# Nextomics/NextPolish2

Measured on AMD Instinct MI355X. Metric: polished reference Mbp/s (whole node) at 30x HiFi + k21/k31; FASTA identical to oracle, higher is better.
Workload: dtype u8

## Files before the change

### nextpolish2_amd/csrc/np2_batch.cpp

```cpp
#include "../../include/np2.h"
#include "np2_ctx.hpp"

#include <atomic>
#include <climits>
#include <cstring>
#include <condition_variable>
#include <mutex>
#include <thread>
#include <pthread.h>

#include <linux/futex.h>
#include <sys/syscall.h>
#include <unistd.h>

using namespace np2;

namespace {

struct Job {
    np2_contig *contig = nullptr;
    const np2_opts_t *opts = nullptr;
    uint8_t **out_bases = nullptr;
    uint32_t **out_pos = nullptr;
    uint64_t *out_len = nullptr;
    uint32_t *out_span = nullptr;
    int *rc = nullptr;
};

}

struct np2_batch {
    np2_ctx *parent = nullptr;
    int device = 0;
    hipStream_t stream = nullptr;
    std::vector<np2_ctx *> slots;
    std::vector<Recorder> recs;
    std::vector<std::thread> workers;
    std::string err;

    std::mutex mu;
    std::condition_variable cv_start, cv_done;
    uint64_t job_gen = 0;
    std::vector<Job> jobs;
    int n_running = 0;
    bool quit = false;

    std::mutex sync_mu;
    int n_active = 0, n_waiting = 0;
    std::atomic<uint32_t> flush_gen{0};
    std::atomic<bool> failed{false};
    std::string fail_msg;

    uint32_t *done_host = nullptr, *done_dev = nullptr;
    uint32_t done_seq = 0;
    std::atomic<uint32_t> issued_seq{0};
    std::atomic<uint32_t> done_pub{0};
    std::atomic<bool> spinner{false};
    double t_issued_last = 0;
    uint32_t wait_logged_seq = 0;

    bool time_diff = false;
    std::vector<std::pair<hipEvent_t, hipEvent_t>> diff_events;
    size_t diff_used = 0;
    float last_diff_ms = 0;
    int last_diff_launches = 0;
    uint64_t stat_launches = 0, stat_cmds = 0, stat_flushes = 0;
    double t_last_end = 0, ms_host = 0, ms_issue = 0, ms_wait = 0;
    std::vector<double> flush_log;
    double call_ms = 0, tail_ms = 0;
};

namespace {

inline void wait_generation(std::atomic<uint32_t> &gen, uint32_t seen) {
    static const double spin_us = getenv("NP2_BATCH_SPIN_US") ? atof(getenv("NP2_BATCH_SPIN_US")) : (wait_naps() ? 0.0 : 5.0);
    const double t_end = now_ms() + spin_us * 1e-3;
    for (;;) {
        for (int i = 0; i < 64; ++i) {
            if (gen.load(std::memory_order_acquire) != seen) return;
            __builtin_ia32_pause();
        }
        if (now_ms() >= t_end) break;
    }
    while (gen.load(std::memory_order_acquire) == seen)
        (void)syscall(SYS_futex, reinterpret_cast<uint32_t *>(&gen), FUTEX_WAIT_PRIVATE, seen, nullptr, nullptr, 0);
}
inline void publish_generation(std::atomic<uint32_t> &gen, uint32_t next) {
    gen.store(next, std::memory_order_release);
    (void)syscall(SYS_futex, reinterpret_cast<uint32_t *>(&gen), FUTEX_WAKE_PRIVATE, INT_MAX, nullptr, nullptr, 0);
}

__device__ __forceinline__ void k_flush_done(const uint32_t np2_bid, const uint32_t np2_nb, uint32_t *__restrict__ word, uint32_t seq) {
    if (threadIdx.x == 0) {
        __threadfence_system();
        __hip_atomic_store(word, seq, __ATOMIC_RELEASE, __HIP_MEMORY_SCOPE_SYSTEM);
    }
}

void flush(np2_batch *b) {
    const int n = (int)b->recs.size();
    const double t_begin = now_ms();
    double t_issued = t_begin;
    std::vector<size_t> idx(n, 0);
    hipStream_t s = b->stream;
    Recorder *saved = tl_recorder();
    tl_recorder() = nullptr;
    try {
        for (;;) {
            bool any = false;
            for (int i = 0; i < n; ++i) {
                auto &q = b->recs[i].q;
                while (idx[i] < q.size() && !q[idx[i]].kd) {
                    q[idx[i]].fn(s);
                    ++idx[i];
                    ++b->stat_cmds;
                }
                any |= idx[i] < q.size();
            }
            if (!any) break;
            const KernelDesc *best = nullptr;
            int best_n = 0, best_defer = 0;
            static constexpr size_t LOOKAHEAD = 8;
            for (int i = 0; i < n; ++i) {
                auto &q = b->recs[i].q;
                if (idx[i] >= q.size()) continue;
                const KernelDesc *kd = q[idx[i]].kd;
                bool seen = false;
                for (int j = 0; j < i && !seen; ++j)
                    seen = idx[j] < b->recs[j].q.size() && b->recs[j].q[idx[j]].kd == kd;
                if (seen) continue;
                int c = 0, defer = 0;
                for (int j = 0; j < n; ++j) {
                    auto &qj = b->recs[j].q;
                    if (idx[j] >= qj.size()) continue;
                    if (qj[idx[j]].kd == kd) {
                        ++c;
                        continue;
                    }
                    for (size_t k = idx[j] + 1; k < qj.size() && k <= idx[j] + LOOKAHEAD; ++k)
                        if (qj[k].kd == kd) {
                            ++defer;
                            break;
                        }
                }
                if (!best || defer < best_defer || (defer == best_defer && c > best_n)) best = kd, best_n = c, best_defer = defer;
            }
            uint32_t grids[MAXB];
            const void *args[MAXB];
            int m = 0;
            const bool timed = b->time_diff && strcmp(best->name, "k_diff_reads") == 0;
            auto issue = [&]() {
                if (!m) return;
                if (timed) {
                    if (b->diff_used == b->diff_events.size()) {
                        hipEvent_t e0 = nullptr, e1 = nullptr;
                        HIPCHK(hipEventCreate(&e0));
                        HIPCHK(hipEventCreate(&e1));
                        b->diff_events.push_back({e0, e1});
                    }
                    HIPCHK(hipEventRecord(b->diff_events[b->diff_used].first, s));
                }
                best->launch(s, m, grids, args);
                if (timed) {
                    HIPCHK(hipEventRecord(b->diff_events[b->diff_used].second, s));
                    ++b->diff_used;
                }
                ++b->stat_launches;
                m = 0;
            };
            for (int i = 0; i < n; ++i) {
                auto &r = b->recs[i];
                if (idx[i] >= r.q.size() || r.q[idx[i]].kd != best) continue;
                grids[m] = r.q[idx[i]].grid;
                args[m] = r.arena.data() + r.q[idx[i]].arg_off;
                ++m;
                ++idx[i];
                ++b->stat_cmds;
                if (m == best->max_batch) issue();
            }
            issue();
        }
        HIPCHK(hipGetLastError());
        const uint32_t seq = ++b->done_seq;
        NP2_LAUNCH(k_flush_done, 1, 64, s, b->done_dev, seq);
        t_issued = now_ms();
        b->issued_seq.store(seq, std::memory_order_release);
    } catch (const std::exception &ex) {
        b->fail_msg = ex.what();
        b->failed.store(true);
        (void)hipStreamSynchronize(s);
        for (np2_ctx *cx : b->slots) cx->lb_dirty = true, cx->h2d_inflight = false;
    }
    tl_recorder() = saved;
    for (auto &r : b->recs) r.clear();
    ++b->stat_flushes;
    b->ms_host += t_begin - b->t_last_end;
    b->ms_issue += t_issued - t_begin;
    b->flush_log.push_back(t_begin - b->t_last_end);
    b->flush_log.push_back(t_issued - t_begin);
    b->flush_log.push_back(0.0);
    b->t_last_end = t_issued;
    b->t_issued_last = t_issued;
}

void wait_done(np2_batch *b, uint32_t seq) {
    for (;;) {
        const uint32_t pub = b->done_pub.load(std::memory_order_acquire);
        if ((int32_t)(pub - seq) >= 0 || b->failed.load()) break;
        bool expected = false;
        if (b->spinner.compare_exchange_strong(expected, true)) {
            uint64_t spins = 0;
            uint32_t cur;
            HostWait hw;
            while ((int32_t)((cur = __atomic_load_n(b->done_host, __ATOMIC_ACQUIRE)) - seq) < 0) {
                if (b->failed.load()) break;
                if ((++spins & (wait_naps() ? 0xFFu : 0xFFFFu)) == 0) {
                    hipError_t e = hipStreamQuery(b->stream);
                    if (e != hipSuccess && e != hipErrorNotReady) {
                        b->fail_msg = std::string("device error during a batch flush: ") + hipGetErrorString(e);
                        b->failed.store(true);
                        break;
                    }
                    if (e == hipSuccess && (int32_t)(__atomic_load_n(b->done_host, __ATOMIC_ACQUIRE) - seq) < 0) {
                        b->fail_msg = "batch flush completed without posting";
                        b->failed.store(true);
                        break;
                    }
                }
                hw.pause();
            }
            b->spinner.store(false);
            publish_generation(b->done_pub, b->failed.load() ? pub + 1 : cur);
            if (b->failed.load()) return;
            continue;
        }
        wait_generation(b->done_pub, pub);
    }
    if (b->failed.load()) return;
    std::lock_guard<std::mutex> l(b->sync_mu);
    if (b->wait_logged_seq != seq && b->issued_seq.load() == seq && !b->flush_log.empty()) {
        const double t = now_ms();
        b->wait_logged_seq = seq;
        b->ms_wait += t - b->t_issued_last;
        b->flush_log.back() = t - b->t_issued_last;
        b->t_last_end = t;
    }
}

void group_sync(Recorder *r, bool need_done) {
    np2_batch *b = (np2_batch *)r->group;
    uint32_t my_gen;
    bool flushed = false;
    {
        std::lock_guard<std::mutex> l(b->sync_mu);
        my_gen = b->flush_gen.load(std::memory_order_relaxed);
        if (++b->n_waiting == b->n_active) {
            flush(b);
            b->n_waiting = 0;
            publish_generation(b->flush_gen, my_gen + 1);
            flushed = true;
        }
    }
    if (!flushed) wait_generation(b->flush_gen, my_gen);
    if (need_done && !b->failed.load()) wait_done(b, b->issued_seq.load(std::memory_order_acquire));
    if (b->failed.load()) throw Np2Error(NP2_E_DEVICE, "batch flush failed: " + b->fail_msg);
}

void leave_wave(np2_batch *b, Recorder *r) {
    std::lock_guard<std::mutex> l(b->sync_mu);
    if (!r->q.empty()) {
        np2_ctx *cx = b->slots[r->slot];
        cx->lb_dirty = true;
        cx->h2d_inflight = false;
    }
    r->clear();
    --b->n_active;
    if (b->n_active > 0 && b->n_waiting == b->n_active) {
        const uint32_t g = b->flush_gen.load(std::memory_order_relaxed);
        flush(b);
        b->n_waiting = 0;
        publish_generation(b->flush_gen, g + 1);
    }
}

void worker_main(np2_batch *b, int slot) {
    (void)hipSetDevice(b->device);
    (void)pthread_setname_np(pthread_self(), "np2-slot");
    uint64_t seen = 0;
    for (;;) {
        Job job;
        {
            std::unique_lock<std::mutex> l(b->mu);
            b->cv_start.wait(l, [&] { return b->quit || b->job_gen != seen; });
            if (b->quit) return;
            seen = b->job_gen;
            job = b->jobs[slot];
        }
        if (!job.contig) continue;
        Recorder *r = &b->recs[slot];
        tl_recorder() = r;
        int rc = np2_polish_resident(b->slots[slot], job.contig, job.opts, job.out_bases, job.out_pos, job.out_len);
        tl_recorder() = nullptr;
        for (auto &g : r->graveyard)
            dev_release_idle(g.first, (g.second >> 63) ? 0 : g.second, (g.second >> 63) ? (g.second & ~(1ull << 63)) : 0);
        r->graveyard.clear();
        leave_wave(b, r);
        if (rc == NP2_OK && job.out_span) (void)np2_last_span(b->slots[slot], &job.out_span[0], &job.out_span[1]);
        *job.rc = rc;
        {
            std::lock_guard<std::mutex> l(b->mu);
            if (--b->n_running == 0) b->cv_done.notify_all();
        }
    }
}

auto batch_sink(np2_batch *b) {
    return [b](int, const std::string &msg) { b->err = msg; };
}

}

extern "C" {

int np2_batch_create(np2_batch_t **out, np2_ctx_t *parent, int n_slots) {
    if (!out || !parent || n_slots < 1 || n_slots > 256) return NP2_E_ARG;
    *out = nullptr;
    return abi_guard([&] {
        std::unique_ptr<np2_batch, void (*)(np2_batch_t *)> b(new np2_batch(), np2_batch_destroy);
        b->parent = parent;
        b->device = parent->device;
        HIPCHK(hipSetDevice(b->device));
        HIPCHK(hipStreamCreateWithFlags(&b->stream, hipStreamNonBlocking));
        HIPCHK(hipHostMalloc((void **)&b->done_host, 256 * (size_t)(n_slots + 1), hipHostMallocMapped | hipHostMallocCoherent));
        memset(b->done_host, 0, 256 * (size_t)(n_slots + 1));
        HIPCHK(hipHostGetDevicePointer((void **)&b->done_dev, b->done_host, 0));
        b->recs.resize(n_slots);
        b->jobs.resize(n_slots);
        for (int i = 0; i < n_slots; ++i) {
            np2_ctx *cx = ctx_create_slot(parent, b->stream, b->done_host + 64 * (size_t)(i + 1), b->done_dev + 64 * (size_t)(i + 1));
            b->slots.push_back(cx);
            b->recs[i].group = b.get();
            b->recs[i].slot = i;
            b->recs[i].sync_fn = &group_sync;
        }
        for (int i = 0; i < n_slots; ++i) b->workers.emplace_back(worker_main, b.get(), i);
        *out = b.release();
        return NP2_OK;
    }, [parent](int, const std::string &msg) { parent->err = msg; });
}

void np2_batch_destroy(np2_batch_t *b) {
    if (!b) return;
    {
        std::lock_guard<std::mutex> l(b->mu);
        b->quit = true;
    }
    b->cv_start.notify_all();
    for (auto &t : b->workers) t.join();
    (void)hipSetDevice(b->device);
    if (b->stream) (void)hipStreamSynchronize(b->stream);
    {
        DevSyncScope idle;
        for (np2_ctx *cx : b->slots) np2_ctx_destroy(cx);
    }
    for (auto &e : b->diff_events) {
        (void)hipEventDestroy(e.first);
        (void)hipEventDestroy(e.second);
    }
    if (b->done_host) (void)hipHostFree(b->done_host);
    if (b->stream) (void)hipStreamDestroy(b->stream);
    delete b;
}

int np2_batch_set_priority(np2_batch_t *b, int high) {
    if (!b) return NP2_E_ARG;
    return abi_guard([&] {
        HIPCHK(hipSetDevice(b->device));
        int least = 0, greatest = 0;
        HIPCHK(hipDeviceGetStreamPriorityRange(&least, &greatest));
        HIPCHK(hipStreamSynchronize(b->stream));
        hipStream_t s = nullptr;
        HIPCHK(hipStreamCreateWithPriority(&s, hipStreamNonBlocking, high ? greatest : least));
        (void)hipStreamDestroy(b->stream);
        b->stream = s;
        for (np2_ctx *cx : b->slots) ctx_slot_set_stream(cx, s);
        return NP2_OK;
    }, batch_sink(b));
}

int np2_batch_slots(np2_batch_t *b) { return b ? (int)b->slots.size() : 0; }
np2_ctx_t *np2_batch_slot_ctx(np2_batch_t *b, int slot) {
    return (b && slot >= 0 && slot < (int)b->slots.size()) ? b->slots[slot] : nullptr;
}
const char *np2_batch_last_error(np2_batch_t *b) { return b ? b->err.c_str() : "null batch"; }
int np2_batch_set_sink(np2_batch_t *b, int slot, void *device_ptr, uint64_t cap) {
    if (!b || slot < 0 || slot >= (int)b->slots.size()) return NP2_E_ARG;
    b->slots[slot]->sink_dst = (uint8_t *)device_ptr;
    b->slots[slot]->sink_cap = device_ptr ? cap : 0;
    return NP2_OK;
}

int np2_batch_polish(np2_batch_t *b, np2_contig_t *const *contigs, int n, const np2_opts_t *opts, uint8_t **out_bases,
                     uint32_t **out_pos, uint64_t *out_len, uint32_t *out_span, int *rcs) {
    if (!b || !contigs || n < 0 || !opts || !out_len || !rcs) return NP2_E_ARG;
    return abi_guard([&] {
        const int S = (int)b->slots.size();
        int worst = NP2_OK;
        b->diff_used = 0;
        b->flush_log.clear();
        b->t_last_end = now_ms();
        const double t_call0 = b->t_last_end;
        for (int w0 = 0; w0 < n; w0 += S) {
            const int m = std::min(S, n - w0);
            {
                std::lock_guard<std::mutex> l(b->mu);
                for (int i = 0; i < S; ++i) {
                    Job j;
                    if (i < m) {
                        j.contig = contigs[w0 + i];
                        j.opts = opts;
                        j.out_bases = out_bases ? &out_bases[w0 + i] : nullptr;
                        j.out_pos = out_pos ? &out_pos[w0 + i] : nullptr;
                        j.out_len = &out_len[w0 + i];
                        j.out_span = out_span ? &out_span[2 * (w0 + i)] : nullptr;
                        j.rc = &rcs[w0 + i];
                    }
                    b->jobs[i] = j;
                }
                b->n_running = m;
                {
                    std::lock_guard<std::mutex> l2(b->sync_mu);
                    b->n_active = m;
                    b->n_waiting = 0;
                    b->failed.store(false);
                }
                ++b->job_gen;
            }
            b->cv_start.notify_all();
            {
                std::unique_lock<std::mutex> l(b->mu);
                b->cv_done.wait(l, [&] { return b->n_running == 0; });
            }
            for (int i = 0; i < m; ++i)
                if (rcs[w0 + i] != NP2_OK) {
                    worst = rcs[w0 + i];
                    b->err = std::string("contig ") + std::to_string(w0 + i) + ": " + np2_last_error(b->slots[i]);
                }
        }
        b->call_ms = now_ms() - t_call0;
        b->tail_ms = now_ms() - b->t_last_end;
        if (b->time_diff) {
            b->last_diff_ms = 0;
            b->last_diff_launches = (int)b->diff_used;
            for (size_t i = 0; i < b->diff_used; ++i) {
                float ms = 0;
                (void)hipEventSynchronize(b->diff_events[i].second);
                (void)hipEventElapsedTime(&ms, b->diff_events[i].first, b->diff_events[i].second);
                b->last_diff_ms += ms;
            }
        }
        return worst;
    }, batch_sink(b));
}

void np2_batch_set_timing(np2_batch_t *b, int enable) {
    if (b) b->time_diff = enable != 0;
}
int np2_batch_last_diff_ms(np2_batch_t *b, float *ms, int *launches) {
    if (!b || !ms || !launches) return NP2_E_ARG;
    *ms = b->last_diff_ms;
    *launches = b->last_diff_launches;
    return NP2_OK;
}
int np2_batch_last_call_ms(np2_batch_t *b, double *total_ms, double *tail_ms) {
    if (!b || !total_ms || !tail_ms) return NP2_E_ARG;
    *total_ms = b->call_ms;
    *tail_ms = b->tail_ms;
    return NP2_OK;
}
int np2_batch_flush_log(np2_batch_t *b, const double **log) {
    if (!b || !log) return 0;
    *log = b->flush_log.data();
    return (int)(b->flush_log.size() / 3);
}
int np2_batch_stats(np2_batch_t *b, uint64_t *launches, uint64_t *commands, uint64_t *flushes) {
    if (!b || !launches || !commands || !flushes) return NP2_E_ARG;
    *launches = b->stat_launches;
    *commands = b->stat_cmds;
    *flushes = b->stat_flushes;
    return NP2_OK;
}
}
```

### nextpolish2_amd/csrc/np2_cand.hip

```cpp
#include "np2_common.hpp"
#include "np2_kernels.hpp"
#include "np2_blockscan.hpp"
#include "np2_lookback.hpp"

namespace np2 {

template <int MODE>
__device__ __forceinline__ void k_scan_small(const uint32_t np2_bid, const uint32_t np2_nb, const uint32_t *__restrict__ in, uint32_t *__restrict__ out,
                                                     uint32_t n_host, const uint32_t *__restrict__ n_dev,
                                                     uint32_t *__restrict__ total_out, bool write_end) {
    __shared__ uint32_t sh[16];
    const uint32_t n = n_dev ? min(*n_dev, n_host) : n_host;
    uint32_t total;
    if (MODE == 2) {
        total = block_scan_array<OpMinI32>(
            n, sh, [&](uint32_t i) { return in[i]; },
            [&](uint32_t i, uint32_t pre, uint32_t v) { out[i] = OpMinI32::apply(pre, v); });
    } else {
        total = block_scan_array<OpAdd>(
            n, sh, [&](uint32_t i) { return in[i]; },
            [&](uint32_t i, uint32_t pre, uint32_t v) { out[i] = MODE == 0 ? pre : pre + v; });
    }
    if (threadIdx.x == 0) {
        if (MODE == 0 && write_end) out[n] = total;
// ... 103 lines not shown
    if (n > c) n -= c, col = 8, m = (uint32_t)(m64 >> 32);
    c = (uint32_t)__builtin_popcount(m & 0xFFFFu);
    if (n > c) n -= c, col += 4, m >>= 16;
    c = (uint32_t)__builtin_popcount(m & 0xFFu);
    if (n > c) n -= c, col += 2, m >>= 8;
    c = (uint32_t)__builtin_popcount(m & 0xFu);
    if (n > c) col += 1;
    return col;
}

__device__ uint32_t cand_measure(const CandCtx &cx, uint32_t r, const np2_read_t &rd, uint64_t ck_off, uint32_t start,
                                 uint32_t end, uint32_t &col_start) {
    uint32_t col_ck, t_ck;
    cand_anchor(cx, r, rd, ck_off, start, col_ck, t_ck);
    col_start = col_ck;
    if (end < t_ck) return 0;
    const uint32_t want_s = (start > t_ck ? start - t_ck : 0u) + 1;
    const uint32_t want_e = end + 1 - t_ck + 1;
    const uint8_t *base = cx.nib + rd.nib_off;
    const uint32_t n_cols = rd.n_cols;
    uint32_t seen = 0, len = 0;
    bool started = false;
    uint4 win = make_uint4(0, 0, 0, 0);
    uint32_t win_blk = 0xFFFFFFFFu;
    const uint64_t N1 = 0x1111111111111111ULL;
    for (uint32_t wi = col_ck >> 4;; ++wi) {
        const uint32_t c0 = wi << 4;
        if (c0 >= n_cols) break;
        if ((wi >> 1) != win_blk) {
            win_blk = wi >> 1;
            win = *reinterpret_cast<const uint4 *>(base + ((size_t)win_blk << 4));
        }
        const uint32_t r0 = (wi & 1) ? win.z : win.x, r1 = (wi & 1) ? win.w : win.y;
        const uint64_t w = (uint64_t)(((r0 & 0x0F0F0F0Fu) << 4) | ((r0 >> 4) & 0x0F0F0F0Fu)) |
                           ((uint64_t)(((r1 & 0x0F0F0F0Fu) << 4) | ((r1 >> 4) & 0x0F0F0F0Fu)) << 32);
        uint64_t valid = N1;
        if (c0 < col_ck) valid &= ~((1ULL << (4 * (col_ck - c0))) - 1ULL);
        if (n_cols - c0 < 16) valid &= (1ULL << (4 * (n_cols - c0))) - 1ULL;
        uint64_t nonins = (~(w >> 3)) & valid;
        if (c0 == 0) nonins |= valid & 1ULL;
        const uint64_t x = (w & 0x7777777777777777ULL) ^ 0x4444444444444444ULL;
        const uint64_t nongap = (x | (x >> 1) | (x >> 2)) & valid;
        const uint32_t cn = (uint32_t)__builtin_popcountll(nonins);
        uint32_t lo = 0, hi = 16;
        bool done = false;
        if (!started && seen + cn >= want_s) {
            lo = nth_col16(nonins, want_s - seen);
            col_start = c0 + lo;
            started = true;
        }
        if (seen + cn >= want_e) {
            hi = nth_col16(nonins, want_e - seen);
            done = true;
        }
        if (started) {
            uint64_t m = nongap;
            if (lo) m &= ~((1ULL << (4 * lo)) - 1ULL);
            if (hi < 16) m &= (1ULL << (4 * hi)) - 1ULL;
            len += (uint32_t)__builtin_popcountll(m);
        }
        seen += cn;
        if (done) break;
    }
    return started ? len : 0u;
}

struct NibReader {
    const uint8_t *base;
    uint64_t w;
    uint32_t wbase;
    __device__ __forceinline__ uint8_t get(uint32_t c) {
        const uint32_t b = c & ~15u;
        if (b != wbase) {
            const uint2 v = *reinterpret_cast<const uint2 *>(base + (b >> 1));
            const uint32_t x = ((v.x & 0x0F0F0F0Fu) << 4) | ((v.x >> 4) & 0x0F0F0F0Fu);
            const uint32_t y = ((v.y & 0x0F0F0F0Fu) << 4) | ((v.y >> 4) & 0x0F0F0F0Fu);
            w = (uint64_t)x | ((uint64_t)y << 32);
            wbase = b;
        }
        return (uint8_t)((w >> (4 * (c & 15))) & 15);
    }
};

__device__ void cand_write(const CandCtx &cx, uint32_t r, const np2_read_t &rd, uint32_t pj, uint32_t g, uint32_t col, uint32_t t,
                           uint32_t len, uint8_t *__restrict__ seq_out, uint64_t *kmer_out) {
    const uint8_t *base = cx.nib + rd.nib_off;
    const uint32_t limit = cx.lq_end[pj] + cx.ksize;
    bool have_kmer = false;
    if (col + cx.ksize <= rd.n_cols) {
        const uint32_t k = cx.ksize, W0 = col >> 4, sh = (col & 15) * 4;
        auto ld = [&](uint32_t W) -> uint64_t {
            const uint2 v = *reinterpret_cast<const uint2 *>(base + ((size_t)W << 3));
            const uint32_t x = ((v.x & 0x0F0F0F0Fu) << 4) | ((v.x >> 4) & 0x0F0F0F0Fu);
            const uint32_t y = ((v.y & 0x0F0F0F0Fu) << 4) | ((v.y >> 4) & 0x0F0F0F0Fu);
            return (uint64_t)x | ((uint64_t)y << 32);
        };
        const uint64_t x0 = ld(W0), x1 = ld(W0 + 1), x2 = ld(W0 + 2);
        uint64_t lo = sh ? (x0 >> sh) | (x1 << (64 - sh)) : x0, hi = sh ? (x1 >> sh) | (x2 << (64 - sh)) : x1;
        auto nmask = [](uint32_t n) -> uint64_t { return n >= 16 ? ~0ULL : ((1ULL << (4 * n)) - 1ULL); };
        const uint64_t N1 = 0x1111111111111111ULL;
        const uint32_t avail = min(32u, rd.n_cols - col);
        const uint64_t a_lo = nmask(avail), a_hi = avail > 16 ? nmask(avail - 16) : 0ULL;
        const uint64_t ng_lo = ~(lo >> 2) & N1 & a_lo, ng_hi = ~(hi >> 2) & N1 & a_hi;
        const uint32_t c_lo = (uint32_t)__builtin_popcountll(ng_lo);
        if (c_lo + (uint32_t)__builtin_popcountll(ng_hi) >= k) {
            uint32_t kk = k, C = 0;
            uint64_t m = ng_lo;
            if (kk > c_lo) kk -= c_lo, C = 16, m = ng_hi;
            uint32_t c = (uint32_t)__builtin_popcount((uint32_t)m);
            if (kk > c) kk -= c, C += 8, m >>= 32;
            uint32_t m32 = (uint32_t)m;
            c = (uint32_t)__builtin_popcount(m32 & 0xFFFFu);
            if (kk > c) kk -= c, C += 4, m32 >>= 16;
            c = (uint32_t)__builtin_popcount(m32 & 0xFFu);
            if (kk > c) kk -= c, C += 2, m32 >>= 8;
            c = (uint32_t)__builtin_popcount(m32 & 0xFu);
            if (kk > c) C += 1;
            const uint64_t u_lo = nmask(C + 1), u_hi = C + 1 > 16 ? nmask(C + 1 - 16) : 0ULL;
            const uint64_t hi4_lo = (lo >> 2) & N1 & u_lo, hi4_hi = (hi >> 2) & N1 & u_hi;
            const bool plain = (((lo | (lo >> 1)) & hi4_lo) | ((hi | (hi >> 1)) & hi4_hi)) == 0;
            const uint64_t r_lo = nmask(C) & ~0xFULL, r_hi = C > 16 ? nmask(C - 16) : 0ULL;
            const uint32_t ins = (uint32_t)__builtin_popcountll(lo & r_lo & 0x8888888888888888ULL) +
                                 (uint32_t)__builtin_popcountll(hi & r_hi & 0x8888888888888888ULL);
            const uint32_t steps = C ? C - 1 : 0u;
            if (plain && t + (steps - ins) <= limit) {
                lo &= u_lo, hi &= u_hi;
                uint64_t g_lo = hi4_lo, g_hi = hi4_hi;
                while (g_lo | g_hi) {
                    if (g_lo) {
                        const uint64_t below = (g_lo & (0 - g_lo)) - 1;
                        lo = (lo & below) | (((lo >> 4) | (hi << 60)) & ~below);
                        g_lo = ((g_lo >> 4) | (g_hi << 60)) & ~below;
                        hi >>= 4;
                        g_hi >>= 4;
                    } else {
                        const uint64_t below = (g_hi & (0 - g_hi)) - 1;
                        hi = (hi & below) | ((hi >> 4) & ~below);
                        g_hi = (g_hi >> 4) & ~below;
                    }
                }
                auto squeeze = [](uint64_t x) -> uint64_t {
                    uint64_t y = x & 0x3333333333333333ULL;
                    y = (y | (y >> 2)) & 0x0F0F0F0F0F0F0F0FULL;
                    y = (y | (y >> 4)) & 0x00FF00FF00FF00FFULL;
                    y = (y | (y >> 8)) & 0x0000FFFF0000FFFFULL;
                    return (y | (y >> 16)) & 0xFFFFFFFFULL;
                };
                const uint64_t mask = (1ULL << (2 * (uint64_t)k)) - 1;
                const uint64_t codes = (squeeze(lo) | (squeeze(hi) << 32)) & mask;
                uint64_t rb = __builtin_bitreverse64(codes);
                rb = ((rb >> 1) & 0x5555555555555555ULL) | ((rb & 0x5555555555555555ULL) << 1);
                const uint64_t fw = rb >> (64 - 2 * k), rv = ~codes & mask;
                *kmer_out = yak_hash64(fw < rv ? fw : rv, mask);
                have_kmer = true;
            }
        }
    }
    if (!have_kmer) {
        NibReader nr{base, 0, 0xFFFFFFFFu};
        const uint64_t ksize = cx.ksize, shift = 2 * (ksize - 1), mask = (1ULL << (2 * ksize)) - 1;
        uint64_t fw = 0, rv = 0, l = 0;
        for (uint32_t c = col; c < rd.n_cols && l < ksize; ++c) {
            const uint8_t nb = nr.get(c);
            if (c != col && !(nb & 8)) ++t;
            const uint8_t q = nb & 7;
            if (q != 4) {
                fw = ((fw << 2) | (uint64_t)q) & mask;
// ... 301 lines not shown
        n_blk, sh, [&](uint32_t i) { return blk_sum[2 * n_blk + i]; }, [&](uint32_t, uint32_t, uint32_t) {});
    if (threadIdx.x == 0) {
        cand_off[n_reg] = ta;
        reg_soff[n_reg] = tb;
        *n_cand = ta;
        *n_bytes = tb;
        *grow = tc;
    }
}

__device__ __forceinline__ void k_cand_offsets_lb(const uint32_t np2_bid, const uint32_t np2_nb, Lookback lb, uint32_t n_blocks, const uint32_t *__restrict__ blk_sum,
                                                         uint32_t n_blk, uint32_t n_reg, uint32_t *__restrict__ blk_coff,
                                                         uint32_t *__restrict__ blk_soff, uint32_t *__restrict__ cand_off,
                                                         uint32_t *__restrict__ reg_soff, uint32_t *__restrict__ n_cand,
                                                         uint32_t *__restrict__ n_bytes, uint32_t *__restrict__ grow,
                                                         uint32_t *__restrict__ err) {
    __shared__ uint32_t sh[8];
    const uint32_t bid = lb_block_id(lb, sh);
    const uint32_t i0 = (bid * 256 + threadIdx.x) * 4;
    uint32_t a[4], b[4], sa = 0, sb = 0;
#pragma unroll
    for (uint32_t k = 0; k < 4; ++k) {
        a[k] = i0 + k < n_blk ? blk_sum[i0 + k] : 0u;
        b[k] = i0 + k < n_blk ? blk_sum[n_blk + i0 + k] : 0u;
        sa += a[k];
        sb += b[k];
    }
    uint32_t ta, tb, pa, pb;
    uint32_t ra = block_excl_scan<OpAdd, 4>(sa, sh, ta);
    uint32_t rb = block_excl_scan<OpAdd, 4>(sb, sh, tb);
    lb_exclusive2(lb, bid, ta, tb, sh, err, pa, pb);
    ra += pa, rb += pb;
#pragma unroll
    for (uint32_t k = 0; k < 4; ++k)
        if (i0 + k < n_blk) {
            blk_coff[i0 + k] = ra;
            blk_soff[i0 + k] = rb;
            ra += a[k];
            rb += b[k];
        }
    if (bid == n_blocks - 1 && threadIdx.x == 255) {
        cand_off[n_reg] = ra;
        reg_soff[n_reg] = rb;
        *n_cand = ra;
        *n_bytes = rb;
    }
    if (bid == 0) {
        uint32_t c = 0, tc;
        for (uint32_t i = threadIdx.x; i < n_blk; i += 256) c += blk_sum[2 * n_blk + i];
        (void)block_excl_scan<OpAdd, 4>(c, sh, tc);
        if (threadIdx.x == 0) *grow = tc;
    }
}

static constexpr uint32_t MERGE_LB_BLOCKS = 32;
__device__ __forceinline__ void k_lq_merge_scan_lb(const uint32_t np2_bid, const uint32_t np2_nb, Lookback lb, const uint32_t *__restrict__ raw_start,
                                                   const uint32_t *__restrict__ raw_end, const uint32_t *__restrict__ n_raw, uint32_t n_host,
                                                   uint32_t *__restrict__ headflag, uint32_t *__restrict__ hidx, uint32_t *__restrict__ err) {
    __shared__ uint32_t sh[16];
    const uint32_t bid = lb_block_id(lb, sh);
    const uint32_t n = min(*n_raw, n_host);
    const uint32_t seg = ((n + MERGE_LB_BLOCKS - 1) / MERGE_LB_BLOCKS + 1023u) & ~1023u;
    const uint32_t lo = min(bid * seg, n), hi = min(lo + seg, n);
    auto flag = [&](uint32_t j) { return (j >= 1 && raw_end[j] >= raw_start[j - 1]) ? 0u : 1u; };
    uint32_t cnt = 0;
    for (uint32_t j = lo + threadIdx.x; j < hi; j += 1024) cnt += flag(j);
    uint32_t total, pre, dummy;
    (void)block_excl_scan<OpAdd, 16>(cnt, sh, total);
    lb_exclusive2(lb, bid, total, 0u, sh, err, pre, dummy);
    uint32_t carry = pre;
    for (uint32_t j0 = lo; j0 < hi; j0 += 1024) {
        const uint32_t j = j0 + threadIdx.x;
        const uint32_t v = j < hi ? flag(j) : 0u;
        uint32_t tot;
        const uint32_t ex = block_excl_scan<OpAdd, 16>(v, sh, tot);
        if (j < hi) {
            hidx[j] = carry + ex;
            headflag[j] = v;
        }
        carry += tot;
    }
}

__device__ __forceinline__ void k_region_write(const uint32_t np2_bid0, const uint32_t np2_nb, CandCtx cx, uint32_t n_reg, const uint32_t *__restrict__ kept_read,
                                                      const uint32_t *__restrict__ kept_len,
                                                      const uint32_t *__restrict__ kept_col,
                                                      const uint32_t *__restrict__ reg_ncand,
                                                      const uint32_t *__restrict__ reg_bytes,
                                                      const uint32_t *__restrict__ blk_coff,
                                                      const uint32_t *__restrict__ blk_soff,
                                                      uint32_t *__restrict__ cand_off, uint32_t *__restrict__ reg_soff,
                                                      uint32_t cand_cap,
                                                      uint32_t seq_cap, uint32_t *__restrict__ cand_order,
                                                      uint64_t *__restrict__ cand_kmer, uint32_t *__restrict__ cand_seq_off,
                                                      uint8_t *__restrict__ cand_seq) {
    const uint32_t np2_bid = xcd_order(np2_bid0, np2_nb);
    __shared__ __attribute__((aligned(4))) uint8_t s_str[RM_REG][CLEAN_MAX_LEN];
    __shared__ uint64_t s_km[RM_REG];
    __shared__ uint32_t s_so[RM_REG][64];
    __shared__ uint32_t s_oc[RM_REG];
    __shared__ uint32_t s_q[4][RM_RPW * 64];
    const uint32_t lane = threadIdx.x & 63, wv = (uint32_t)__builtin_amdgcn_readfirstlane((int)(threadIdx.x >> 6));
    const uint32_t g0 = (np2_bid * 4 + wv) * RM_RPW, mb0 = g0 / 4;
    uint32_t nq = 0;
    uint32_t oc = 0, ob = 0;
    if (g0 < n_reg) oc = blk_coff[mb0], ob = blk_soff[mb0];
    uint32_t clean_h = 0;
    uint32_t my_len[RM_RPW], my_so[RM_RPW], my_ci[RM_RPW];
    bool my_clean[RM_RPW];
    uint32_t n[RM_RPW], rb[RM_RPW], st[RM_RPW], ln0[RM_RPW];
#pragma unroll
    for (uint32_t h = 0; h < RM_RPW; ++h) {
        const uint32_t g = g0 + h;
        n[h] = 0, rb[h] = 0, st[h] = 0, ln0[h] = 0;
        if (g < n_reg) n[h] = reg_ncand[g], rb[h] = reg_bytes[g], st[h] = cx.lq_start[g], ln0[h] = cx.lq_end[g] - st[h] + 1;
    }
    uint32_t len[RM_RPW], col[RM_RPW], rd_[RM_RPW], refc[RM_RPW];
#pragma unroll
    for (uint32_t h = 0; h < RM_RPW; ++h) {
        const size_t ks = (size_t)(g0 + h) * LQSEQ_MAX_CAN_COUNT + lane;
        const bool act = lane < n[h];
        len[h] = act ? kept_len[ks] : 0u;
        col[h] = act ? kept_col[ks] : 0u;
        rd_[h] = act ? kept_read[ks] : 0u;
        const uint32_t p = st[h] + lane;
        refc[h] = (n[h] && lane < ln0[h] && ln0[h] <= CLEAN_MAX_LEN) ? cx.refnib[p >> 3] >> (4 * (p & 7)) : 0u;
    }
#pragma unroll
    for (uint32_t h = 0; h < RM_RPW; ++h) {
        const uint32_t g = g0 + h, slot = wv * RM_RPW + h;
        my_len[h] = 0, my_so[h] = 0, my_ci[h] = 0, my_clean[h] = false;
        if (g >= n_reg) continue;
        if (g == n_reg - 1 && lane == 0 && cand_off[n_reg] < cand_cap) cand_seq_off[cand_off[n_reg]] = reg_soff[n_reg];
        if (lane == 0) {
            cand_off[g] = oc;
            reg_soff[g] = ob;
            s_oc[slot] = oc;
        }
        const bool act = lane < n[h];
        const uint32_t so = ob + wave_excl(len[h]);
        const uint32_t ci = oc + lane;
        const bool ok = act && ci < cand_cap && (uint64_t)so + len[h] <= seq_cap;
        if (ok) {
            cand_order[ci] = rd_[h];
            cand_seq_off[ci] = so;
        }
        const bool clean = ok && col[h] == CAND_CLEAN;
        const uint64_t cm = __ballot(clean);
        const bool queued = ok && (!clean || (lane == 0 && rd_[h] == 0));
        my_len[h] = len[h], my_so[h] = so, my_ci[h] = ci, my_clean[h] = clean && !queued;
        s_so[slot][lane] = so;
        if (cm) {
            clean_h |= 1u << h;
            if (lane < ln0[h]) s_str[slot][lane] = (uint8_t)((0x54474341u >> (8 * (refc[h] & 3))) & 0xFFu);
        }
        const uint64_t dq = __ballot(queued);
        if (queued) s_q[wv][nq + lanes_below(dq)] = (slot << 6) | lane;
        nq += (uint32_t)__builtin_popcountll(dq);
        oc += n[h];
        ob += rb[h];
    }
    wave_lds_sync();
    for (uint32_t e = lane; e < nq; e += 64) {
        const uint32_t w = s_q[wv][e], slot = w >> 6, li = w & 63;
        const uint32_t g = (np2_bid * 4 + slot / RM_RPW) * RM_RPW + slot % RM_RPW;
        const size_t ks = (size_t)g * LQSEQ_MAX_CAN_COUNT + li;
        const uint32_t r = kept_read[ks], len = kept_len[ks];
        uint32_t col = kept_col[ks];
        const ReadInfo ri = cx.rinfo[r];
        const np2_read_t rd = rinfo_read(ri);
        const uint32_t t0 = max(cx.lq_start[g], rd.aln_t_s);
        if (col == CAND_CLEAN) col = t0;
        const uint32_t ci = s_oc[slot] + li;
        uint64_t km;
        cand_write(cx, r, rd, ri.pj, g, col, t0, len, cand_seq + s_so[slot][li], &km);
        cand_kmer[ci] = km;
        if (li == 0 && r == 0) s_km[slot] = km;
    }
    wave_lds_sync();
#pragma unroll
    for (uint32_t h = 0; h < RM_RPW; ++h) {
        if (!((clean_h >> h) & 1u)) continue;
        const uint32_t slot = wv * RM_RPW + h;
        if (my_clean[h]) {
            cand_kmer[my_ci[h]] = s_km[slot];
            typedef uint32_t u32_any __attribute__((aligned(1)));
            uint8_t *dst = cand_seq + my_so[h];
            const uint32_t L4 = my_len[h] & ~3u;
            for (uint32_t j = 0; j < L4; j += 4) *reinterpret_cast<u32_any *>(dst + j) = *reinterpret_cast<const uint32_t *>(&s_str[slot][j]);
            for (uint32_t j = L4; j < my_len[h]; ++j) dst[j] = s_str[slot][j];
        }
    }
}

void launch_scan_small_excl(hipStream_t s, const uint32_t *in, uint32_t *out, uint32_t n, const uint32_t *n_dev,
                            uint32_t *total_out, bool write_end) {
    NP2_LAUNCH(k_scan_small<0>, dim3(1), 1024, s, in, out, n, n_dev, total_out, write_end);
}
void launch_scan_lb_excl(hipStream_t s, const Lookback &lb, const uint32_t *in, uint32_t *out, uint32_t n, bool write_end,
                          uint32_t *err) {
    const uint32_t nb = scan_lb_blocks(n);
    NP2_LAUNCH(k_scan_lb_excl, dim3(nb), SCAN_LB_THREADS, s, lb, nb, in, out, n, write_end, err);
}
void launch_scan_lb_popc(hipStream_t s, const Lookback &lb, const uint32_t *bits, uint32_t *out, uint32_t n_words, uint32_t *err) {
    const uint32_t nb = scan_lb_blocks((uint64_t)n_words + 1);
    NP2_LAUNCH(k_scan_lb_popc, dim3(nb), SCAN_LB_THREADS, s, lb, nb, bits, out, n_words + 1, false, err);
}
uint32_t scan_lb_blocks(uint64_t n) { return (uint32_t)std::max<uint64_t>(1, (n + SCAN_LB_BLOCK - 1) / SCAN_LB_BLOCK); }
void launch_scan_small_incl(hipStream_t s, const int32_t *in, int32_t *out, uint32_t n, const uint32_t *n_dev) {
    NP2_LAUNCH(k_scan_small<1>, dim3(1), 1024, s, (const uint32_t *)in, (uint32_t *)out, n, n_dev, (uint32_t *)nullptr, false);
}
void launch_scan_small_min(hipStream_t s, const int32_t *in, int32_t *out, uint32_t n, const uint32_t *n_dev) {
    NP2_LAUNCH(k_scan_small<2>, dim3(1), 1024, s, (const uint32_t *)in, (uint32_t *)out, n, n_dev, (uint32_t *)nullptr, false);
}
static CandCtx mk_cand(const CandPtrs &c) {
    return CandCtx{c.reads, c.nib,    c.ck_off, c.ckpt,        c.lq_start, c.lq_end, c.pj,
                   c.pcount, c.alive, c.rinfo, c.tile_rd_off, c.tile_rd, c.n_tiles,  c.ksize,
                   c.rec_key, c.rec_read, c.tile_n, c.rec_pidx, c.bucket_cap, c.refnib, c.L};
}
void launch_region_measure(hipStream_t s, const CandPtrs &c, uint32_t n_reg, uint32_t *kept_read, uint32_t *kept_len,
                           uint32_t *kept_col, uint32_t *reg_ncand, uint32_t *reg_bytes, uint32_t *reg_maxlen,
                           uint32_t *blk_sum) {
    if (n_reg)
        NP2_LAUNCH_WAVES(k_region_measure, RM_WAVES, dim3((n_reg + RM_REG - 1) / RM_REG), 256, s,
                         mk_cand(c), n_reg, kept_read, kept_len, kept_col, reg_ncand, reg_bytes, reg_maxlen, blk_sum);
}
uint32_t cand_offsets_blocks(uint32_t n_reg) { return ((n_reg + 3) / 4 + 1023) / 1024; }
void launch_cand_offsets(hipStream_t s, const uint32_t *blk_sum, uint32_t n_reg, uint32_t *blk_coff, uint32_t *blk_soff,
                         uint32_t *cand_off, uint32_t *reg_soff, uint32_t *n_cand, uint32_t *n_bytes, uint32_t *grow,
                         const Lookback *lb, uint32_t *err) {
    if (lb)
        NP2_LAUNCH(k_cand_offsets_lb, dim3(cand_offsets_blocks(n_reg)), 256, s, *lb, cand_offsets_blocks(n_reg), blk_sum, (n_reg + 3) / 4, n_reg, blk_coff, blk_soff, cand_off, reg_soff, n_cand, n_bytes, grow, err);
    else
        NP2_LAUNCH(k_cand_offsets, dim3(1), 1024, s, blk_sum, (n_reg + 3) / 4, n_reg, blk_coff, blk_soff, cand_off, reg_soff, n_cand, n_bytes, grow);
}
void launch_lq_merge_scan_lb(hipStream_t s, const Lookback &lb, const uint32_t *raw_start, const uint32_t *raw_end, const uint32_t *n_raw,
                             uint32_t n_host, uint32_t *headflag, uint32_t *hidx, uint32_t *err) {
    NP2_LAUNCH(k_lq_merge_scan_lb, dim3(MERGE_LB_BLOCKS), 1024, s, lb, raw_start, raw_end, n_raw, n_host, headflag, hidx, err);
}
uint32_t lq_merge_lb_blocks() { return MERGE_LB_BLOCKS; }
void launch_region_write(hipStream_t s, const CandPtrs &c, uint32_t n_reg, const uint32_t *kept_read,
                         const uint32_t *kept_len, const uint32_t *kept_col, const uint32_t *reg_ncand,
                         const uint32_t *reg_bytes, const uint32_t *blk_coff, const uint32_t *blk_soff, uint32_t *cand_off,
                         uint32_t *reg_soff, uint32_t cand_cap, uint32_t seq_cap, uint32_t *cand_order, uint64_t *cand_kmer,
                         uint32_t *cand_seq_off, uint8_t *cand_seq) {
    if (n_reg)
        NP2_LAUNCH(k_region_write, dim3((n_reg + RM_REG - 1) / RM_REG), 256, s, mk_cand(c), n_reg, kept_read, kept_len, kept_col, reg_ncand, reg_bytes, blk_coff, blk_soff, cand_off, reg_soff, cand_cap, seq_cap, cand_order, cand_kmer, cand_seq_off, cand_seq);
}

}
```

### nextpolish2_amd/csrc/np2_host.cpp

```cpp
#include "../../include/np2.h"
#include "np2_common.hpp"
#include "np2_kernels.hpp"
#include "np2_ctx.hpp"
#include "np2_phase_host.hpp"

#include <algorithm>
#include <atomic>
#include <thread>
#include <chrono>
#include <cstdio>
#include <cstdlib>
#include <cstring>
#include <map>
#include <mutex>
#include <stdexcept>
#include <string>
#include <unordered_map>
#include <unordered_set>
#include <future>
#include <functional>
#include <vector>

using namespace np2;

// ... 130 lines not shown
            off_own.assign(off, off + R + 1);
            edges_own.assign(edges, edges + off[R]);
            off = off_own.data(), edges = edges_own.data();
        }
        if (!view_key) return;
        pair_key.assign(view_key, view_key + view_n);
        pair_cnt.assign(view_cnt, view_cnt + view_n);
        view_key = nullptr, view_cnt = nullptr, view_n = 0;
    }
    std::vector<uint32_t> first_key;
    std::vector<int32_t> ref_w;
    std::vector<uint8_t> ref_seen, bad;
    const uint8_t *d_bad = nullptr;
    bool key_added = false;
};

bool vote_rows_from_pairs(VoteData &vd, bool use_all) {
    const uint32_t R = vd.R;
    const uint64_t *k = vd.keys();
    const uint32_t *cn = vd.cnts();
    const uint64_t np = vd.n_pairs();
    std::vector<uint32_t> n_lo(R, 0), n_up(R, 0);
    uint32_t nokey = 0;
    auto listed = [&](uint64_t i, uint32_t &a, uint32_t &b) {
        a = (uint32_t)(k[i] >> 32), b = (uint32_t)k[i];
        if (a >= R || b >= R || vd.first_key[a] == 0xFFFFFFFFu || vd.first_key[b] == 0xFFFFFFFFu) return false;
        return use_all || !(vd.bad[a] | vd.bad[b]);
    };
    for (uint64_t i = 0; i < np; ++i) {
        uint32_t a = (uint32_t)(k[i] >> 32), b = (uint32_t)k[i];
        if (b <= a || b - a - 1 >= EDGE_BAND || (i && k[i - 1] >= k[i])) return false;
        if (a >= R || b >= R || vd.first_key[a] == 0xFFFFFFFFu || vd.first_key[b] == 0xFFFFFFFFu) ++nokey;
        if (listed(i, a, b)) ++n_lo[b], ++n_up[a];
    }
    vd.off_own.assign((size_t)R + 1, 0);
    std::vector<uint32_t> cur_lo(R), cur_up(R);
    for (uint32_t v = 0; v < R; ++v) {
        cur_lo[v] = vd.off_own[v], cur_up[v] = vd.off_own[v] + n_lo[v];
        vd.off_own[v + 1] = cur_up[v] + n_up[v];
    }
    vd.edges_own.resize(vd.off_own[R]);
    for (uint64_t i = 0; i < np; ++i) {
        uint32_t a, b;
        if (!listed(i, a, b)) continue;
        const int32_t same = (int32_t)(cn[i] & 0xFFFFu), neg = (int32_t)(cn[i] >> 16);
        const float w = (float)(neg >= 3 ? -neg : same - neg);
        vd.edges_own[cur_lo[b]++] = phase::Graph::Edge(a, w);
        vd.edges_own[cur_up[a]++] = phase::Graph::Edge(b, w);
    }
    vd.off = vd.off_own.data(), vd.edges = vd.edges_own.data(), vd.n_nokey = nokey;
    return true;
}

void vote_collect(np2_ctx *cx, np2_contig *c, PassCounts &pc, bool asref, bool use_all, int pass, uint32_t own_lo,
                  uint32_t own_hi, VoteData &vd, bool wide = false, uint64_t key_add = 0) {
    hipStream_t s = cx->stream;
    const uint32_t R = c->R, n_reg = pc.n_reg;
    RegionTables rt = region_tables(cx, n_reg);
    uint32_t NE = 0, NU = 0;
    vd = VoteData();
    vd.R = R;
    {
        EventTimer t(cx, "vote_phase");
        cx->reg_lable.ensure(n_reg + 2);
        cx->grp.ensure((size_t)pc.NC_cap + 2);
        cx->ecount.ensure(n_reg + 2);
        cx->eoff.ensure(std::max<size_t>(n_reg + 2, (size_t)c->L + 2));
        const size_t RP = ((size_t)R + 63) & ~(size_t)63;
        const size_t band_words = (size_t)R * EDGE_BAND;
        const size_t b_v = RP * 10, b_off = (((size_t)R + 2) * 4 + 15) & ~(size_t)15;
        uint8_t *vbuf;
        uint32_t *row_off;
        if (wide) {
            cx->votebuf.ensure(b_v);
            cx->band_off.ensure((size_t)R + 2);
            vbuf = cx->votebuf.p, row_off = cx->band_off.p;
        } else {
            cx->votepack.ensure(b_v + b_off + band_words * 2 * sizeof(phase::Graph::Edge) + 64);
            vbuf = cx->votepack.p, row_off = (uint32_t *)(cx->votepack.p + b_v);
        }
        uint32_t *v_first = (uint32_t *)vbuf;
        int32_t *v_refw = (int32_t *)(vbuf + RP * 4);
        uint8_t *v_seen = vbuf + RP * 8, *v_bad = vbuf + RP * 9;
        op_fill(cx, v_first, 0xFF, RP * 4);
        op_fill(cx, v_refw, 0, RP * 6);
        launch_vote_phase(s, rt, asref, use_all, cx->lq_start.p, own_lo, own_hi, cx->reg_lable.p, cx->grp.p, cx->ecount.p,
                          v_refw, v_seen, v_bad, v_first, cx->scal.p + S_ERR);
        exclusive_total_n(cx, cx->ecount.p, cx->eoff.p, n_reg);
        launch_vote_counts(s, v_first, v_bad, R, cx->scal.p + S_M1);
        cx->band.ensure(band_words + 4);
        cx->band_n.ensure((size_t)R + 2);
        op_fill(cx, cx->scal.p + S_M3, 0, 4);
        launch_edges_row(s, rt, cx->grp.p, cx->ecount.p, cx->pj.p, cx->pcount.p, cx->alive.p, R, cx->band.p, cx->band_n.p,
                         cx->scal.p + S_M3);
        if (wide) {
            exclusive_total_n(cx, cx->band_n.p, row_off, R);
            cx->ekey.ensure(band_words + 2);
            cx->eval.ensure(band_words + 2);
            launch_band_emit(s, cx->band.p, R, row_off, cx->ekey.p, cx->eval.p, cx->scal.p + S_NRAW, key_add);
        } else {
            cx->row_cnt.ensure((size_t)R + 2);
            launch_vote_rows_count(s, cx->band.p, cx->band_n.p, v_bad, use_all, R, cx->row_cnt.p, cx->scal.p + S_NOKEY);
            exclusive_total_n(cx, cx->row_cnt.p, row_off, R);
            launch_vote_rows_emit(s, cx->band.p, cx->band_n.p, v_bad, use_all, v_first, R, row_off, cx->votepack.p + b_v + b_off,
                                  cx->scal.p + S_NRAW, cx->scal.p + S_NOKEY);
        }
    }
    const size_t RP = ((size_t)R + 63) & ~(size_t)63;
    const size_t b_v = RP * 10, b_off = (((size_t)R + 2) * 4 + 15) & ~(size_t)15;
    auto per_read = [&](const uint8_t *vb) {
        vd.first_key.assign((const uint32_t *)vb, (const uint32_t *)vb + R);
        vd.ref_w.assign((const int32_t *)(vb + RP * 4), (const int32_t *)(vb + RP * 4) + R);
        vd.ref_seen.assign(vb + RP * 8, vb + RP * 8 + R);
        vd.bad.assign(vb + RP * 9, vb + RP * 9 + R);
    };
    bool far = false, have_per_read = false;
    {
        std::vector<uint32_t> sc;
        uint8_t *pin = nullptr;
        const size_t EB = sizeof(phase::Graph::Edge);
        static_assert(sizeof(phase::Graph::Edge) == 8 && alignof(phase::Graph::Edge) <= 8, "an edge is {u32 neighbour, f32 weight}");
        const uint32_t likely = (uint32_t)std::min<size_t>((size_t)R * EDGE_BAND * 2, std::max<size_t>((size_t)R * 128, 1u << 15));
        if (wide) {
            sc = fetch_scal(cx, cx->scal.p + S_M0, cx->eoff.p + n_reg);
        } else {
            pin = (uint8_t *)cx->pin_d2h.ensure(b_v + b_off + (size_t)likely * EB + 64);
            const uint32_t seq = ++cx->mbox_seq;
            launch_post(cx->stream, cx->scal.p, S_COUNT, cx->mbox_dev, seq, cx->scal.p + S_M0, cx->eoff.p + n_reg, nullptr, nullptr,
                        nullptr, nullptr, nullptr, nullptr, nullptr, nullptr);
            op_d2h(cx, pin, cx->votepack.p, b_v + b_off);
            launch_copy_counted(cx->stream, (uint32_t *)(pin + b_v + b_off), (const uint32_t *)(cx->votepack.p + b_v + b_off),
                                (const uint32_t *)(cx->votepack.p + b_v) + R, likely * (uint32_t)(EB / 4), (uint32_t)(EB / 4));
            op_sync(cx);
            if (__atomic_load_n(&cx->mbox_host[0], __ATOMIC_ACQUIRE) != seq)
                throw Np2Error(NP2_E_DEVICE, "mailbox not posted after a synchronisation");
            sc.assign(cx->mbox_host + 1, cx->mbox_host + 1 + S_COUNT);
        }
        check_region_err(cx, sc[S_ERR]);
        pc.resolve(sc);
        NE = sc[S_M0];
        if (!cx->trace && sc[S_M1] == 0 && sc[S_M2] == 0) {
            if (NE) throw Np2Error(NP2_E_DEVICE, "internal: pair edges without voting reads");
            return;
        }
        NU = sc[S_NRAW];
        far = sc[S_M3] != 0 || cx->hooks.edge_sort;
        if (!wide) cx->timing.host.push_back({far ? "vote_sort" : "vote_rows", 1.0f});
        if (!wide) {
            per_read(pin);
            have_per_read = true;
            vd.d_bad = cx->votepack.p + RP * 9;
            if (!far) {
                if (NU > likely) {
                    pin = (uint8_t *)cx->pin_d2h.ensure(b_v + b_off + (size_t)NU * EB + 64);
                    op_d2h(cx, pin, cx->votepack.p, b_v + b_off + (size_t)NU * EB);
                    op_sync(cx);
                }
                vd.off = (const uint32_t *)(pin + b_v), vd.edges = (const phase::Graph::Edge *)(pin + b_v + b_off);
                vd.n_nokey = sc[S_NOKEY];
                if (vd.off[R] != NU) throw Np2Error(NP2_E_DEVICE, "internal: vote rows and edge count disagree");
            }
        }
    }
    vd.any = true;
    if (NE && far) {
        {
            EventTimer t(cx, "vote_phase");
            cx->ekey.ensure(NE + 2);
            cx->ekey_s.ensure(NE + 2);
            cx->eval.ensure(NE + 2);
            cx->eval_s.ensure(NE + 2);
            cx->eflag.ensure(NE + 2);
            cx->eidx.ensure(NE + 2);
            cx->ew.ensure(NE + 2);
            cx->tmp.ensure(prim_temp_bytes((size_t)NE + 2));
            launch_edges_write(s, rt, cx->reg_lable.p, cx->grp.p, cx->ecount.p, cx->eoff.p, cx->ekey.p, cx->eval.p);
            unsigned rbits = 1;
            while ((1ull << rbits) < (uint64_t)R + 1) ++rbits;
            prim_op(cx, [=](hipStream_t st) {
                if (prim_sort_pairs_u64_u32(st, cx->tmp.p, cx->tmp.cap, cx->ekey.p, cx->ekey_s.p, cx->eval.p, cx->eval_s.p, NE,
                                            32 + rbits))
                    throw Np2Error(NP2_E_DEVICE, "rocprim edge sort failed");
            });
            launch_edge_reduce(s, cx->ekey_s.p, cx->eval_s.p, NE, cx->eflag.p, (uint32_t *)cx->ew.p);
            exclusive_total(cx, cx->eflag.p, cx->eidx.p, NE);
            launch_edge_compact(s, cx->ekey_s.p, cx->eflag.p, cx->eidx.p, (const uint32_t *)cx->ew.p, NE, cx->ekey.p,
                                cx->eval.p, cx->scal.p + S_NRAW);
            NU = fetch_scal(cx)[S_NRAW];
        }
    } else if (!NE) {
        NU = 0;
    }
    if (wide || far) {
        const size_t b_key = ((size_t)NU * 8 + 15) & ~(size_t)15, b_w = ((size_t)NU * 4 + 15) & ~(size_t)15;
        const size_t b_pr = have_per_read ? 0 : b_v;
        uint8_t *pin = (uint8_t *)cx->pin_d2h.ensure(b_key + b_w + b_pr + 64);
        if (tl_recorder()) {
            cx->votepack2.ensure(b_key + b_w + b_pr + 64);
            op_copy_d2d(cx, cx->votepack2.p, cx->ekey.p, (size_t)NU * 8);
            op_copy_d2d(cx, cx->votepack2.p + b_key, cx->eval.p, (size_t)NU * 4);
            if (b_pr) op_copy_d2d(cx, cx->votepack2.p + b_key + b_w, cx->votebuf.p, b_pr);
            op_d2h(cx, pin, cx->votepack2.p, b_key + b_w + b_pr);
        } else {
            op_d2h(cx, pin, cx->ekey.p, (size_t)NU * 8);
            op_d2h(cx, pin + b_key, cx->eval.p, (size_t)NU * 4);
            if (b_pr) op_d2h(cx, pin + b_key + b_w, cx->votebuf.p, b_pr);
        }
        op_sync(cx);
        vd.view_key = (const uint64_t *)pin, vd.view_cnt = (const uint32_t *)(pin + b_key), vd.view_n = NU;
        vd.key_added = wide && !far;
        if (b_pr) {
            per_read(pin + b_key + b_w);
            if (wide) vd.d_bad = cx->votebuf.p + RP * 9;
        }
    }
// ... 554 lines not shown
            fprintf(stderr, "\n");
        }
        const bool wide = n_tiles >= 2048;
        Lookback lb{};
        if (wide) lb = next_lookback(cx, tile_scan_blocks(n_tiles));
        launch_tile_offsets(s, cx->tile_nn.p, cx->tile_nr.p, n_tiles, cx->tile_noff.p, cx->tile_roff.p, M_p, n_lq,
                            cx->scal.p + S_BEST, S_NLQ + 1 - S_BEST, wide ? &lb : nullptr, cx->scal.p + S_ERR,
                            (const long long *)cx->tile_gain.p, (unsigned long long *)(cx->scal.p + S_PFGAIN0));
        launch_pf_compact(s, n_tiles, cx->pf_slots.p, cx->tile_scan.p, cx->tile_nn.p, cx->tile_noff.p, cx->tile_roff.p,
                          cx->cns_pos.p, cx->cns_base.p, cx->cns_cls.p, cx->lq_nothead.p, cx->lq_list.p, cb.lq_cap,
                          cx->scal.p + S_ERR, cx->scal.p + S_PF, cx->scal.p + S_PFOUT, cx->scal.p + S_NBAD, cx->scal.p + S_NBAD2);
    }
    lq_regions_issue(cx, cb, M_p, n_lq);
}

void pass_front_issue(np2_ctx *cx, np2_contig *c, uint32_t T, int pass, bool force_unfused = false) {
    cx->front_fused = !force_unfused && front_can_fuse(cx);
    if (!cx->front_fused || cx->trace) {
        uint32_t n_nodes = 0, n_runs = 0;
        {
            WallTimer w(cx, "wall_graph");
            build_graph(cx, c, T, n_nodes, n_runs);
        }
        trace_graph(cx, c, pass, n_nodes);
        if (!cx->front_fused) {
            consensus_and_regions_issue(cx, c, n_nodes, n_runs, T);
            return;
        }
    }
    pass_front_fused_issue(cx, c, T);
}
void consensus_and_regions_finish(np2_ctx *cx, np2_contig *c, uint32_t T, int pass, uint32_t &M, uint32_t &n_reg, bool whole_contig = true) {
    const uint32_t *M_p = cx->eoff.p + c->L;
    std::vector<uint32_t> sc = fetch_scal(cx, cx->scal.p + S_M0, M_p);
    if (cx->front_fused) {
        const int64_t total = (int64_t)(((uint64_t)sc[S_PFGAIN1] << 32) | sc[S_PFGAIN0]);
        const int64_t end_rel = (int64_t)(((uint64_t)sc[S_PFEND1] << 32) | sc[S_PFEND0]);
        const bool negative = end_rel <= SCORE_NEG / 2 || total + end_rel < 0;
        if (sc[S_PFOUT] & PF_NEED_BIG) cx->pf_big = true;
        if ((sc[S_PFOUT] & PF_REDO) || negative) {
            ++cx->front_redos;
            cx->timing.host.push_back({"front_redo", 1.0f});
            pass_front_issue(cx, c, T, pass, true);
            sc = fetch_scal(cx, cx->scal.p + S_M0, M_p);
        }
    }
    check_region_err(cx, sc[S_ERR]);
    if (!cx->front_fused && sc[S_BEST] == 0xFFFFFFFFu && !whole_contig)
        throw Np2Error(NP2_E_UNSUPPORTED,
                       "best path score is negative at the end of a shard (the reference's default node is chosen by the whole "
                       "contig's score): polish this contig unsharded");
    M = sc[S_M0];
    if (M == 0) throw Np2Error(NP2_E_REFPANIC, "reference would panic: empty consensus");
    n_reg = sc[S_NRAW] ? sc[S_NREG] : 0;
}

void extract_candidates(np2_ctx *cx, np2_contig *c, uint32_t n_reg, uint16_t min_kmer_count, int pass,
                        PassCounts &pc) {
    hipStream_t s = cx->stream;
    const uint32_t R = c->R;
    REFPANIC_IF(cx->yaks.empty(), "index out of bounds: opt.yak[0]");
    if ((uint64_t)n_reg * LQSEQ_MAX_CAN_COUNT >= 0xFFFFFFF0ull) throw Np2Error(NP2_E_NOMEM, "too many LQ regions");
    const uint32_t NC_cap = n_reg * LQSEQ_MAX_CAN_COUNT;
    static const uint64_t exact_from = getenv("NP2_CAND_EXACT_FROM") ? strtoull(getenv("NP2_CAND_EXACT_FROM"), nullptr, 10) : (1ull << 28);
    const bool exact_bytes = c->n_cols >= exact_from && !cx->trace;
    uint32_t SB_cap = (uint32_t)std::min<uint64_t>(c->n_cols + 64, 0xFFFFFFF0ull);
    cx->mval.ensure(R + 2);
    cx->smin.ensure(R + 2);
    cx->pj.ensure(R + 2);
    cx->pcount.ensure(R + 2);
    cx->rinfo.ensure(R + 2);
    cx->reg_ncand.ensure(n_reg + 2);
    cx->reg_bytes.ensure(n_reg + 2);
    cx->reg_soff.ensure(n_reg + 2);
    cx->reg_maxlen.ensure(n_reg + 2);
    cx->blk_sum.ensure(3 * ((size_t)n_reg / 4 + 2));
    cx->blk_coff.ensure((size_t)n_reg / 4 + 2);
    cx->blk_soff.ensure((size_t)n_reg / 4 + 2);
    cx->cand_off.ensure(n_reg + 2);
    cx->kept_read.ensure((size_t)NC_cap + 2);
    cx->kept_len.ensure((size_t)NC_cap + 2);
    cx->kept_col.ensure((size_t)NC_cap + 2);
    cx->cand_order.ensure((size_t)NC_cap + 2);
    cx->cand_kmer.ensure((size_t)NC_cap + 2);
    cx->cand_seq_off.ensure((size_t)NC_cap + 2);
    if (!exact_bytes) cx->cand_seq.ensure((size_t)SB_cap + 64);
    cx->kscore.ensure((size_t)NC_cap + 2);
    cx->long_list.ensure((size_t)NC_cap + 2);
    CandPtrs cp{c->reads.p,   c->nib.p,   c->ck_off.p,      c->ckpt.p,    cx->lq_start.p, cx->lq_end.p, cx->pj.p,
                cx->pcount.p, cx->alive.p, cx->rinfo.p, c->tile_rd_off.p, c->tile_rd.p, c->n_tiles, cx->yaks[0].k,
                cx->keys_raw.p, cx->vals_raw.p, cx->tile_n.p,
                (cx->pidx_valid && cx->bucket_cap) ? cx->tile_pidx.p : nullptr, cx->bucket_cap,
                (const uint32_t *)c->refnib.p, c->L};
    {
        EventTimer t(cx, "candidates");
        launch_read_m(s, c->reads.p, R, cx->alive.p, cx->lq_start.p, n_reg, cx->mval.p);
        scan_incl_min(cx, cx->mval.p, cx->smin.p, R);
        launch_pair_count(s, c->reads.p, R, cx->alive.p, cx->lq_start.p, cx->lq_end.p, n_reg, cx->smin.p, cx->pj.p,
                          cx->pcount.p, c->ck_off.p, cx->rinfo.p);
        launch_region_measure(s, cp, n_reg, cx->kept_read.p, cx->kept_len.p, cx->kept_col.p, cx->reg_ncand.p,
                              cx->reg_bytes.p, cx->reg_maxlen.p, cx->blk_sum.p);
        {
            const bool wide = n_reg > 0;
            Lookback lb{};
            if (wide) lb = next_lookback(cx, cand_offsets_blocks(n_reg));
            launch_cand_offsets(s, cx->blk_sum.p, n_reg, cx->blk_coff.p, cx->blk_soff.p, cx->cand_off.p, cx->reg_soff.p,
                                cx->scal.p + S_NC, cx->scal.p + S_SB, cx->scal.p + S_GROW, wide ? &lb : nullptr,
                                cx->scal.p + S_ERR);
        }
        if (exact_bytes) {
            const std::vector<uint32_t> sc = fetch_scal(cx);
            check_region_err(cx, sc[S_ERR]);
            pc.resolve(sc);
            SB_cap = (uint32_t)std::min<uint64_t>((uint64_t)pc.SB + 64, SB_cap);
            cx->cand_seq.ensure((size_t)SB_cap + 64);
        }
        launch_region_write(s, cp, n_reg, cx->kept_read.p, cx->kept_len.p, cx->kept_col.p, cx->reg_ncand.p,
                            cx->reg_bytes.p, cx->blk_coff.p, cx->blk_soff.p, cx->cand_off.p, cx->reg_soff.p, NC_cap + 1,
                            SB_cap, cx->cand_order.p, cx->cand_kmer.p, cx->cand_seq_off.p, cx->cand_seq.p);
    }
    {
        EventTimer t(cx, "kmer_score");
        launch_cand_score(s, cx->yaks[0].dev(), cx->cand_seq_off.p, cx->cand_seq.p, cx->cand_kmer.p, cx->scal.p + S_NC,
                          NC_cap, min_kmer_count, cx->kscore.p, cx->long_list.p, cx->scal.p + S_NLONG);
    }
    pc.n_reg = n_reg;
    pc.NC_cap = NC_cap;
    pc.SB_cap = SB_cap;
    pc.known = exact_bytes;
    if (cx->trace) pc.resolve(fetch_scal(cx));
    trace_region_tables(cx, pass, "cand", pc, false);
}

Cns fetch_cns(np2_ctx *cx, uint32_t M) {
    Cns c;
    c.pos = d2h(cx, cx->cns_pos.p, M);
    c.base = d2h(cx, cx->cns_base.p, M);
    return c;
}

struct ResultOut {
    uint8_t *bases = nullptr;
    uint32_t *pos = nullptr;
    uint64_t len = 0;
    bool want_pos = true;
    bool want_bases = true;
    void release() {
        if (bases) pinned_pool().put(bases), bases = nullptr;
        if (pos) pinned_pool().put(pos), pos = nullptr;
    }
};
void fetch_result(np2_ctx *cx, const uint32_t *dpos, const uint8_t *dbase, const uint32_t *M_p, uint32_t M_cap, ResultOut &r,
                  uint32_t M_likely = 0xFFFFFFFFu) {
    const double t0 = now_ms();
    std::vector<uint32_t> sc;
    if (cx->sink_dst && cx->sink_cap) launch_copy_len(cx->stream, cx->sink_dst, dbase, M_p, 1, cx->sink_cap);
    if (r.want_bases || r.want_pos) {
        const uint32_t seq = ++cx->mbox_seq;
        launch_post(cx->stream, cx->scal.p, S_COUNT, cx->mbox_dev, seq, cx->scal.p + S_M0, M_p, nullptr, nullptr, nullptr, nullptr,
                    nullptr, nullptr, dpos, cx->scal.p + S_M1);
        if (r.want_bases) r.bases = (uint8_t *)pinned_pool().get((size_t)M_cap + 1);
        if (r.want_pos) r.pos = (uint32_t *)pinned_pool().get(((size_t)M_cap + 1) * 4);
        if ((r.want_bases && !r.bases) || (r.want_pos && !r.pos)) throw Np2Error(NP2_E_NOMEM, "pinned result allocation failed");
        uint32_t first = std::min(M_cap, M_likely);
        const bool exact_b = r.want_bases && op_d2h_len(cx, r.bases, dbase, M_p, 1, M_cap);
        const bool exact_p = r.want_pos && op_d2h_len(cx, r.pos, dpos, M_p, 4, (size_t)M_cap * 4);
        if (r.want_bases && !exact_b) op_d2h(cx, r.bases, dbase, first);
        if (r.want_pos && !exact_p) op_d2h(cx, r.pos, dpos, (size_t)first * 4);
        if ((exact_b || !r.want_bases) && (exact_p || !r.want_pos)) first = M_cap;
        op_sync(cx);
        if (__atomic_load_n(&cx->mbox_host[0], __ATOMIC_ACQUIRE) != seq)
            throw Np2Error(NP2_E_DEVICE, "mailbox not posted after a synchronisation");
        sc.assign(cx->mbox_host + 1, cx->mbox_host + 1 + S_COUNT);
        if (sc[S_M0] > first && sc[S_M0] <= M_cap) {
            const uint32_t rest = sc[S_M0] - first;
            if (r.want_bases) op_d2h(cx, r.bases + first, dbase + first, rest);
            if (r.want_pos) op_d2h(cx, r.pos + first, dpos + first, (size_t)rest * 4);
            op_sync(cx);
        }
    } else {
        sc = fetch_scal(cx, cx->scal.p + S_M0, M_p, nullptr, nullptr, nullptr, nullptr, nullptr, nullptr, dpos, cx->scal.p + S_M1);
    }
    check_region_err(cx, sc[S_ERR]);
    const uint32_t M = sc[S_M0];
    if (M == 0) throw Np2Error(NP2_E_REFPANIC, "reference would panic: empty consensus");
    if (M > M_cap) throw Np2Error(NP2_E_DEVICE, "internal: consensus longer than its bound");
    r.len = M;
    cx->last_first_pos = sc[S_M1];
    cx->last_last_pos = sc[S_M2];
    cx->last_dbase = dbase;
    cx->last_dpos = dpos;
    cx->last_len = M;
    if (cx->stage_timing) cx->timing.host.push_back({"wall_fetch_result", (float)(now_ms() - t0)});
}

struct PolishRun {
    np2_ctx *cx = nullptr;
    np2_contig *c = nullptr;
    np2_opts_t o{};
    uint32_t own_lo = 0, own_hi = 0xFFFFFFFFu;
    uint32_t T = 0, pass = 0, M = 0, n_reg = 0;
    bool reuse = false;
    bool front_issued = false;
    uint32_t grow_prev = 0xFFFFFFFFu;
    bool wide_votes = false;
    uint64_t key_add = 0;
    PassCounts pc;
    bool final_pass() const { return pass + 1 == o.iter_count; }
};

void run_begin(PolishRun &r) {
    np2_ctx *cx = r.cx;
    if (r.o.iter_count < 1) throw Np2Error(NP2_E_ARG, "iter_count must be >= 1");
    HIPCHK(hipSetDevice(cx->device));
    cx->trace_items.clear();
    cx->last_dbase = nullptr;
    cx->last_dpos = nullptr;
    cx->scal.ensure(SCAL_TOTAL);
    cx->alive.ensure(r.c->R + 2);
    {
        WallTimer w(cx, "wall_diff");
        run_diff(cx, r.c, r.T);
    }
    launch_init_alive(cx->stream, r.c->reads.p, r.c->R, cx->alive.p);
    r.pass = 0;
    r.reuse = false;
}

void run_pass_front(PolishRun &r) {
    np2_ctx *cx = r.cx;
    np2_contig *c = r.c;
    if (!r.reuse) {
        {
            WallTimer w(cx, "wall_cns_lq");
            if (!r.front_issued) pass_front_issue(cx, c, r.T, (int)r.pass);
            r.front_issued = false;
            consensus_and_regions_finish(cx, c, r.T, (int)r.pass, r.M, r.n_reg, !r.wide_votes);
        }
        if (cx->trace) {
            trace_cns(cx, (int)r.pass, "cns_raw", fetch_cns(cx, r.M));
            trace_put(cx, (int)r.pass, "lq.start", d2h(cx, cx->lq_start.p, r.n_reg));
            trace_put(cx, (int)r.pass, "lq.end", d2h(cx, cx->lq_end.p, r.n_reg));
        }
    }
    if (r.n_reg == 0) return;
    if (!r.reuse) {
        r.pc = PassCounts();
        r.pc.M = r.M;
        WallTimer w(cx, "wall_extract");
        extract_candidates(cx, c, r.n_reg, r.o.min_kmer_count, (int)r.pass, r.pc);
    } else if (r.pc.NC_cap) {
        op_copy_d2d(cx, cx->kscore.p, cx->kscore_saved.p, (size_t)(r.pc.known ? r.pc.NC : r.pc.NC_cap) * 2);
// ... 1192 lines not shown
```

### nextpolish2_amd/csrc/np2_kernels.hip

```cpp
#include "np2_common.hpp"
#include "np2_kernels.hpp"
#include "np2_blockscan.hpp"
#include "np2_nib128.hpp"
#include "../../include/np2.h"

namespace np2 {

__device__ __forceinline__ uint8_t ref_code(const uint8_t *__restrict__ refnib, uint32_t p) {
    return (refnib[p >> 1] >> (4 * (p & 1))) & 7;
}

__device__ __forceinline__ void k_encode_ref(const uint32_t np2_bid, const uint32_t np2_nb, const uint8_t *__restrict__ read0, uint32_t L, uint8_t *__restrict__ refnib,
                             uint32_t nbytes_total, uint32_t stride, uint32_t *__restrict__ err) {
    uint32_t i = np2_bid * blockDim.x + threadIdx.x;
    if (i >= nbytes_total) return;
    uint32_t c0 = 2 * i, c1 = 2 * i + 1;
    uint8_t b = c0 < L ? read0[i] : 0;
    uint8_t hi = c0 < L ? (b >> 4) : 0, lo = c1 < L ? (b & 15) : 0;
    if ((c0 < L && c0 != 0 && (hi & 8)) || (c1 < L && (lo & 8))) atomicOr(err, 1u);
    if (c0 < L && (hi & 7) == 7) atomicOr(err, 1u);
    if (c1 < L && (lo & 7) == 7) atomicOr(err, 1u);
    refnib[i] = (uint8_t)((hi & 7) | ((lo & 7) << 4));
    const uint8_t nx = c1 + 1 < L ? (uint8_t)((read0[i + 1] >> 4) & 7) : (uint8_t)0;
    refnib[stride + i] = (uint8_t)(((hi & 7) << 4) | (lo & 7));
    refnib[2 * (size_t)stride + i] = (uint8_t)(((lo & 7) << 4) | nx);
}

__device__ __forceinline__ void k_post(const uint32_t np2_bid, const uint32_t np2_nb, uint32_t *__restrict__ scal, uint32_t n_scal, uint32_t *__restrict__ mbox, uint32_t seq,
                       uint32_t *__restrict__ dst0, const uint32_t *__restrict__ src0, uint32_t *__restrict__ dst1,
                       const uint32_t *__restrict__ src1, uint32_t *__restrict__ dst2, const uint32_t *__restrict__ src2,
                       uint32_t *__restrict__ dst3, const uint32_t *__restrict__ src3,
                       const uint32_t *__restrict__ ends_of, uint32_t *__restrict__ ends_dst) {
    if (threadIdx.x == 0) {
        if (dst0) *dst0 = *src0;
        if (dst1) *dst1 = *src1;
        if (dst2) *dst2 = *src2;
        if (dst3) *dst3 = *src3;
        if (ends_of) {
            const uint32_t n = *dst0;
            ends_dst[0] = n ? ends_of[0] : 0u;
            ends_dst[1] = n ? ends_of[n - 1] : 0u;
        }
    }
    __threadfence();
    if (threadIdx.x < n_scal)
        mbox[1 + threadIdx.x] = __hip_atomic_load(&scal[threadIdx.x], __ATOMIC_RELAXED, __HIP_MEMORY_SCOPE_AGENT);
    __threadfence_system();
    if (threadIdx.x == 0) __hip_atomic_store(&mbox[0], seq, __ATOMIC_RELEASE, __HIP_MEMORY_SCOPE_SYSTEM);
}
__device__ __forceinline__ void k_fill(const uint32_t np2_bid, const uint32_t np2_nb, uint8_t *__restrict__ p, uint64_t n, uint32_t v4) {
    const uint64_t o = ((uint64_t)np2_bid * 256 + threadIdx.x) * 16;
    if (o >= n) return;
    if ((((uintptr_t)p) & 15) == 0 && o + 16 <= n) {
        *reinterpret_cast<uint4 *>(p + o) = make_uint4(v4, v4, v4, v4);
    } else {
        for (uint64_t i = o; i < min(o + 16, n); ++i) p[i] = (uint8_t)v4;
    }
}
__device__ __forceinline__ void k_copy(const uint32_t np2_bid, const uint32_t np2_nb, uint8_t *__restrict__ dst, const uint8_t *__restrict__ src, uint64_t n) {
    const uint64_t o = ((uint64_t)np2_bid * 256 + threadIdx.x) * 16;
    if (o >= n) return;
    const uintptr_t al = ((uintptr_t)dst) | ((uintptr_t)src);
    if ((al & 15) == 0 && o + 16 <= n) {
        *reinterpret_cast<uint4 *>(dst + o) = *reinterpret_cast<const uint4 *>(src + o);
    } else if ((al & 3) == 0 && o + 16 <= n) {
#pragma unroll
        for (uint32_t q = 0; q < 4; ++q)
            *reinterpret_cast<uint32_t *>(dst + o + 4 * q) = *reinterpret_cast<const uint32_t *>(src + o + 4 * q);
    } else {
        for (uint64_t i = o; i < min(o + 16, n); ++i) dst[i] = src[i];
    }
}
__device__ __forceinline__ void k_copy_len(const uint32_t np2_bid, const uint32_t np2_nb, uint8_t *__restrict__ dst, const uint8_t *__restrict__ src,
                                           const uint32_t *__restrict__ n_dev, uint32_t elem, uint64_t cap) {
    k_copy(np2_bid, np2_nb, dst, src, min((uint64_t)*n_dev * elem, cap));
}
__device__ __forceinline__ void k_copy_counted(const uint32_t np2_bid, const uint32_t np2_nb, uint32_t *__restrict__ dst, const uint32_t *__restrict__ src,
                                               const uint32_t *__restrict__ n_dev, uint32_t cap, uint32_t words_per) {
    const uint32_t n = (uint32_t)min((uint64_t)*n_dev * words_per, (uint64_t)cap);
    const bool wide = ((((uintptr_t)dst) | ((uintptr_t)src)) & 15) == 0;
    for (uint64_t o = ((uint64_t)np2_bid * 256 + threadIdx.x) * 4; o < n; o += (uint64_t)np2_nb * 256 * 4) {
        if (wide && o + 4 <= n) {
            *reinterpret_cast<uint4 *>(dst + o) = *reinterpret_cast<const uint4 *>(src + o);
        } else {
            for (uint64_t i = o; i < min(o + 4, (uint64_t)n); ++i) dst[i] = src[i];
        }
    }
}
__device__ __forceinline__ void k_init_alive(const uint32_t np2_bid, const uint32_t np2_nb, const np2_read_t *__restrict__ reads, uint32_t R, uint8_t *__restrict__ alive) {
    uint32_t r = np2_bid * blockDim.x + threadIdx.x;
    if (r < R) alive[r] = (reads[r].flags & NP2_READ_DROPPED) ? 0 : 1;
}
__device__ __forceinline__ void k_kill_flagged(const uint32_t np2_bid, const uint32_t np2_nb, const uint8_t *__restrict__ flag, uint32_t n, uint8_t *__restrict__ alive) {
    uint32_t i = np2_bid * blockDim.x + threadIdx.x;
    if (i < n && flag[i]) alive[i] = 0;
}
__device__ __forceinline__ void k_kill_reads(const uint32_t np2_bid, const uint32_t np2_nb, const uint32_t *__restrict__ ids, uint32_t n, uint8_t *__restrict__ alive) {
    uint32_t i = np2_bid * blockDim.x + threadIdx.x;
    if (i < n) alive[ids[i]] = 0;
}
__device__ __forceinline__ void k_revive_reads(const uint32_t np2_bid, const uint32_t np2_nb, const uint32_t *__restrict__ ids, uint32_t n, uint8_t *__restrict__ alive) {
    uint32_t i = np2_bid * blockDim.x + threadIdx.x;
    if (i < n) alive[ids[i]] = 1;
}

struct Graph {
    const uint8_t *refnib;
    const uint32_t *node_off;
    NodeArrays nd;
    const int32_t *cov;
    uint32_t L;
    const uint2 *nrec;
    const uint32_t *deep;
};
__device__ __forceinline__ void n0_key(const Graph &g, uint32_t p, uint16_t &bases, uint16_t &delta) {
    const uint8_t c = ref_code(g.refnib, p);
    if (p >= 2) {
        bases = (uint16_t)((ref_code(g.refnib, p - 2) << 8) | (ref_code(g.refnib, p - 1) << 4) | c);
        delta = 0;
    } else if (p == 1) {
        bases = (uint16_t)(0x0F00 | (ref_code(g.refnib, 0) << 4) | c);
        delta = 1;
    } else {
        bases = (uint16_t)(0x4FF0 | c);
        delta = 0;
    }
}
__device__ __forceinline__ uint32_t n0_count(const Graph &g, uint32_t p) {
    uint32_t e0 = 0;
    for (uint32_t i = g.node_off[p]; i < g.node_off[p + 1]; ++i)
    {
        const uint2 rc = g.nrec[i];
        if (node_delta3((uint16_t)rc.x, (uint16_t)(rc.x >> 16)) == 0) e0 += rc.y;
    }
    return (uint32_t)g.cov[p] - e0;
}

__device__ __forceinline__ int64_t early_run_base(const Graph &g, uint32_t a) {
    if (a != 1 && a != 2) return 0;
// ... 1062 lines not shown
        while (atomicCAS((unsigned long long *)&tb[s], (unsigned long long)YAK_EMPTY, (unsigned long long)w) != YAK_EMPTY)
            s = (s + 1) & capm;
        ob[s] = (uint32_t)i;
    }
}

__device__ __forceinline__ void k_lookup(const uint32_t np2_bid, const uint32_t np2_nb, YakDev y, const uint64_t *__restrict__ hashes, uint64_t n, uint16_t min_count,
                         uint16_t *__restrict__ out) {
    uint64_t i = (uint64_t)np2_bid * blockDim.x + threadIdx.x;
    if (i < n) out[i] = yak_get(y, hashes[i], min_count);
}

__device__ __forceinline__ uint16_t wave_score_string_any(const YakDev &y, const uint8_t *__restrict__ s, uint32_t len,
                                                          uint16_t min_count) {
    const uint32_t lane = threadIdx.x & 63;
    const uint32_t k = y.k;
    const uint64_t mask = (1ULL << (2 * (uint64_t)k)) - 1, shift = 2 * ((uint64_t)k - 1);
    uint32_t mn = 0xFFFFFFFFu;
    if (len >= k) {
        for (uint32_t st = lane; st + k <= len; st += 64) {
            uint64_t fw = 0, rv = 0;
            bool ok = true;
            for (uint32_t j = 0; j < k; ++j) {
                const uint64_t c = ascii_to_code(s[st + j]);
                if (c >= 4) {
                    ok = false;
                    break;
                }
                fw = ((fw << 2) | c) & mask;
                rv = (rv >> 2) | ((3ULL ^ c) << shift);
            }
            if (ok) mn = min(mn, (uint32_t)yak_get(y, yak_hash64(fw < rv ? fw : rv, mask), min_count));
        }
    }
    for (int o = 32; o > 0; o >>= 1) mn = min(mn, (uint32_t)__shfl_xor(mn, o));
    return mn == 0xFFFFFFFFu ? (uint16_t)0 : (uint16_t)mn;
}
__device__ __forceinline__ uint16_t wave_score_string(const YakDev &y, const uint8_t *__restrict__ s, uint32_t len,
                                                      uint16_t min_count) {
    const uint32_t lane = threadIdx.x & 63;
    const uint32_t k = y.k;
    const uint64_t mask = (1ULL << (2 * (uint64_t)k)) - 1;
    uint32_t mn = 0xFFFFFFFFu;
    if (len >= k) {
        for (uint32_t st = lane; st + k <= len; st += 64) {
            uint64_t codes = 0, bad = 0;
#pragma unroll
            for (uint32_t wd = 0; wd < 4; ++wd) {
                uint64_t x;
                __builtin_memcpy(&x, s + st + 8 * wd, 8);
                uint64_t c = ((x >> 1) ^ (x >> 2)) & 0x0303030303030303ULL;
                c = (c | (c >> 6)) & 0x000F000F000F000FULL;
                c = (c | (c >> 12)) & 0x000000FF000000FFULL;
                c = (c | (c >> 24)) & 0xFFFFULL;
                codes |= c << (16 * wd);
                uint64_t b = (x >> 3) & 0x0101010101010101ULL;
                b = (b | (b >> 7)) & 0x0003000300030003ULL;
                b = (b | (b >> 14)) & 0x0000000F0000000FULL;
                b = (b | (b >> 28)) & 0xFFULL;
                bad |= b << (8 * wd);
            }
            if ((bad & ((1ULL << k) - 1ULL)) == 0) {
                codes &= mask;
                uint64_t rb = __builtin_bitreverse64(codes);
                rb = ((rb >> 1) & 0x5555555555555555ULL) | ((rb & 0x5555555555555555ULL) << 1);
                const uint64_t fw = rb >> (64 - 2 * k), rv = ~codes & mask;
                mn = min(mn, (uint32_t)yak_get(y, yak_hash64(fw < rv ? fw : rv, mask), min_count));
            }
        }
    }
    for (int o = 32; o > 0; o >>= 1) mn = min(mn, (uint32_t)__shfl_xor(mn, o));
    return mn == 0xFFFFFFFFu ? (uint16_t)0 : (uint16_t)mn;
}

__device__ __forceinline__ void k_score_strings(const uint32_t np2_bid, const uint32_t np2_nb, YakDev y, const uint8_t *__restrict__ strs, const uint64_t *__restrict__ off,
                                uint64_t n, uint16_t min_count, uint16_t *__restrict__ out, uint32_t own_strings) {
    const uint64_t w = ((uint64_t)np2_bid * (blockDim.x >> 6)) + (uint32_t)__builtin_amdgcn_readfirstlane((int)(threadIdx.x >> 6));
    if (w >= n) return;
    const uint16_t sc = own_strings ? wave_score_string(y, strs + off[w], (uint32_t)(off[w + 1] - off[w]), min_count)
                                    : wave_score_string_any(y, strs + off[w], (uint32_t)(off[w + 1] - off[w]), min_count);
    if ((threadIdx.x & 63) == 0) out[w] = sc;
}

__device__ __forceinline__ void k_cand_score(const uint32_t np2_bid, const uint32_t np2_nb, YakDev y, const uint32_t *__restrict__ cand_seq_off, const uint64_t *__restrict__ cand_kmer,
                             const uint32_t *__restrict__ n_cand_p, uint16_t min_count,
                             uint16_t *__restrict__ kscore, uint32_t *__restrict__ long_list,
                             uint32_t *__restrict__ n_long) {
    const uint32_t c = np2_bid * blockDim.x + threadIdx.x;
    const bool live = c < *n_cand_p;
    const uint32_t len = live ? cand_seq_off[c + 1] - cand_seq_off[c] : 0u;
    const bool is_long = live && len > y.k;
    const uint64_t m = __ballot(is_long);
    if (m) {
        const uint32_t lane = threadIdx.x & 63, lead = (uint32_t)__builtin_ctzll(m);
        uint32_t base = 0;
        if (lane == lead) base = atomicAdd(n_long, (uint32_t)__builtin_popcountll(m));
        base = __shfl(base, lead);
        if (is_long) long_list[base + (uint32_t)__builtin_popcountll(m & ((1ULL << lane) - 1ULL))] = c;
    }
    if (!live) return;
    uint16_t sc = 0;
    if (!is_long) {
        const uint64_t km = cand_kmer[c];
        if (km != INVALID_KMER) sc = yak_get(y, km, min_count);
    }
    kscore[c] = sc;
}
__device__ __forceinline__ void k_cand_score_long(const uint32_t np2_bid, const uint32_t np2_nb, YakDev y, const uint32_t *__restrict__ cand_seq_off,
                                  const uint8_t *__restrict__ cand_seq, const uint32_t *__restrict__ long_list,
                                  const uint32_t *__restrict__ n_long, uint16_t min_count,
                                  uint16_t *__restrict__ kscore) {
    const uint32_t nl = *n_long;
    for (uint32_t w = (uint32_t)__builtin_amdgcn_readfirstlane((int)((np2_bid * blockDim.x + threadIdx.x) >> 6)); w < nl; w += (np2_nb * blockDim.x) >> 6) {
        const uint32_t c = long_list[w];
        const uint16_t sc = wave_score_string(y, cand_seq + cand_seq_off[c], cand_seq_off[c + 1] - cand_seq_off[c],
                                              min_count);
        if ((threadIdx.x & 63) == 0) kscore[c] = sc;
    }
}

}

namespace np2 {
static inline dim3 grid1(uint64_t n, uint32_t bs = 256) { return dim3((unsigned)((n + bs - 1) / bs)); }

void launch_encode_ref(hipStream_t s, const uint8_t *read0, uint32_t L, uint8_t *refnib, uint32_t nbytes,
                       uint32_t stride, uint32_t *err) {
    NP2_LAUNCH(k_encode_ref, grid1(nbytes), 256, s, read0, L, refnib, nbytes, stride, err);
}
void launch_post(hipStream_t s, uint32_t *scal, uint32_t n_scal, uint32_t *mbox, uint32_t seq, uint32_t *d0,
                 const uint32_t *s0, uint32_t *d1, const uint32_t *s1, uint32_t *d2, const uint32_t *s2, uint32_t *d3,
                 const uint32_t *s3, const uint32_t *ends_of, uint32_t *ends_dst) {
    NP2_LAUNCH(k_post, dim3(1), 64, s, scal, n_scal, mbox, seq, d0, s0, d1, s1, d2, s2, d3, s3, ends_of, ends_dst);
}
void launch_fill(hipStream_t s, uint8_t *p, uint64_t bytes, uint8_t byte) {
    if (bytes) NP2_LAUNCH(k_fill, grid1((bytes + 15) / 16), 256, s, p, bytes, 0x01010101u * byte);
}
void launch_copy(hipStream_t s, uint8_t *dst, const uint8_t *src, uint64_t bytes) {
    if (bytes) NP2_LAUNCH(k_copy, grid1((bytes + 15) / 16), 256, s, dst, src, bytes);
}
void launch_copy_len(hipStream_t s, uint8_t *dst, const uint8_t *src, const uint32_t *n_dev, uint32_t elem, uint64_t cap_bytes) {
    if (cap_bytes) NP2_LAUNCH(k_copy_len, grid1((cap_bytes + 15) / 16), 256, s, dst, src, n_dev, elem, cap_bytes);
}
void launch_copy_counted(hipStream_t s, uint32_t *dst, const uint32_t *src, const uint32_t *n_dev, uint32_t cap, uint32_t words_per) {
    if (cap) NP2_LAUNCH(k_copy_counted, dim3(std::max<uint32_t>(1, std::min<uint32_t>((cap + 1023) / 1024, 2048))), 256, s, dst, src, n_dev, cap, words_per);
}
void launch_init_alive(hipStream_t s, const np2_read_t *reads, uint32_t R, uint8_t *alive) {
    NP2_LAUNCH(k_init_alive, grid1(R), 256, s, reads, R, alive);
}
void launch_kill_flagged(hipStream_t s, const uint8_t *flag, uint32_t n, uint8_t *alive) {
    if (n) NP2_LAUNCH(k_kill_flagged, grid1(n), 256, s, flag, n, alive);
}
void launch_kill_reads(hipStream_t s, const uint32_t *ids, uint32_t n, uint8_t *alive) {
    if (n) NP2_LAUNCH(k_kill_reads, grid1(n), 256, s, ids, n, alive);
}
void launch_revive_reads(hipStream_t s, const uint32_t *ids, uint32_t n, uint8_t *alive) {
    if (n) NP2_LAUNCH(k_revive_reads, grid1(n), 256, s, ids, n, alive);
}
static Graph mk_graph(const GraphPtrs &gp) { return Graph{gp.refnib, gp.node_off, gp.nd, gp.cov, gp.L, gp.nrec, gp.deep}; }

void launch_dp_short(hipStream_t s, const GraphPtrs &gp, const void *refw, const uint32_t *run_start,
                     const uint32_t *n_runs, uint32_t max_runs, uint32_t *run_end, int64_t *run_gain, uint32_t *emit,
                     uint32_t *path_begin, uint64_t *path, uint32_t *dp_list, uint32_t *n_dp_list) {
    if (max_runs)
        NP2_LAUNCH(k_dp_bt_short, dim3(std::min<uint32_t>((max_runs + 63) / 64, DP_GRID_CAP)), 64, s, run_start, n_runs, mk_graph(gp), (const uint32_t *)refw, run_end, run_gain, emit, path_begin, path, dp_list, n_dp_list);
}
void launch_dp_long(hipStream_t s, const GraphPtrs &gp, const uint32_t *run_start, uint32_t max_runs, const uint2 *nrec,
                    int64_t *nscore, uint32_t *nbesti, uint32_t *n0_besti, uint32_t *run_end, int64_t *last_n0_score,
                    int64_t *run_gain, uint32_t *emit, uint32_t *path_begin, uint64_t *path, uint8_t *run_flag,
                    const uint32_t *dp_list, const uint32_t *n_dp_list) {
    if (!max_runs) return;
    NP2_LAUNCH(k_dp_bt_oct, dim3(std::min<uint32_t>((max_runs + 7) / 8, 2048u)), 64, s, run_start, mk_graph(gp), nrec, nscore, nbesti, n0_besti, run_end, last_n0_score, run_gain, emit, path_begin, path, run_flag, dp_list, n_dp_list);
    NP2_LAUNCH(k_dp_bt_long, dim3(std::min<uint32_t>((max_runs + DP_BLOCK - 1) / DP_BLOCK, 512u)), DP_BLOCK, s, run_start, mk_graph(gp), nrec, nscore, nbesti, n0_besti, run_end, last_n0_score, run_gain, emit, path_begin, path, run_flag, dp_list, n_dp_list);
}
void launch_dp_finish(hipStream_t s, const GraphPtrs &gp, const uint32_t *run_start, const uint32_t *n_runs,
                      const int64_t *nscore, const uint32_t *nbesti, const uint32_t *n0_besti, const int64_t *last_n0_score,
                      unsigned long long *total_gain, uint32_t *blocks_done, uint32_t *best_idx, const int64_t *run_gain,
                      const long long *tile_gain, uint32_t n_tiles, uint32_t *emit, uint32_t *path_begin, uint64_t *path) {
    NP2_LAUNCH(k_dp_finish, dim3(64), 256, s, run_gain, n_runs, tile_gain, n_tiles, total_gain, blocks_done, mk_graph(gp), nscore, last_n0_score, run_start, nbesti, n0_besti, best_idx, emit, path_begin, path);
}
static inline dim3 run_grid(uint32_t bound) { return dim3(std::max<uint32_t>(1, std::min<uint32_t>((bound + 256) / 256, 4096))); }
void launch_bt_write(hipStream_t s, const GraphPtrs &gp, const uint32_t *run_start, const uint32_t *n_runs,
                     uint32_t run_bound, const uint32_t *emit, const uint32_t *eoff, const uint64_t *path,
                     uint32_t *cns_pos, uint8_t *cns_base, uint8_t *cns_cls, uint8_t *lq_nothead, uint32_t *lqc) {
    NP2_LAUNCH(k_cns_write, grid1(gp.L), 256, s, gp.refnib, gp.pflag, emit, eoff, gp.L, cns_pos, cns_base, cns_cls, lq_nothead);
    NP2_LAUNCH(k_cns_runs, run_grid(4 * (uint64_t)run_bound > 0xFFFFFFF0ull ? 0xFFFFFFF0u : 4 * run_bound), 256, s, run_start, n_runs, run_bound, gp.node_off, emit, eoff, path, cns_pos, cns_base, cns_cls, lq_nothead, lqc);
}
void launch_lq_list(hipStream_t s, const GraphPtrs &gp, const uint32_t *run_start, const uint32_t *n_runs,
                    uint32_t run_bound, const uint32_t *emit, const uint32_t *eoff, const uint64_t *path,
                    const uint32_t *lqoff, uint32_t cap, uint32_t *lq_list, uint32_t *err) {
    NP2_LAUNCH(k_lq_list, run_grid(run_bound), 256, s, run_start, n_runs, run_bound, gp.node_off, emit, eoff, path, lqoff, cap, lq_list, err);
}
void launch_default_tail(hipStream_t s, const GraphPtrs &gp, const uint32_t *best_idx, const uint32_t *M_p, uint8_t *cns_base,
                         uint8_t *cns_cls, uint32_t *lq_list, uint32_t *n_lq, uint32_t cap, uint32_t *err) {
    NP2_LAUNCH(k_default_tail, 1, 64, s, best_idx, gp.node_off, gp.pflag, gp.L, M_p, cns_base, cns_cls, lq_list, n_lq, cap, err);
}
static inline dim3 lq_grid(uint32_t cap) { return dim3(std::max<uint32_t>(1, std::min<uint32_t>((cap + 2047) / 2048, 2048))); }
void launch_lq_scan(hipStream_t s, const uint32_t *cns_pos, const uint8_t *cns_base, const uint8_t *cns_cls,
                    const uint32_t *M_p, const uint32_t *lq_list, const uint32_t *n_lq, uint32_t lq_cap, uint8_t *lq_kind,
                    uint32_t *lq_next, uint8_t *lq_nothead, uint32_t *hbits, uint32_t n_hwords, uint32_t *rstart, uint32_t *rend) {
    NP2_LAUNCH(k_lq_scan, lq_grid(std::max(lq_cap, n_hwords / 4)), 256, s, cns_pos, cns_base, cns_cls, M_p, lq_list, n_lq, lq_cap, lq_kind, lq_next, lq_nothead, hbits, n_hwords);
    NP2_LAUNCH(k_lq_region, lq_grid(lq_cap), 256, s, cns_pos, cns_base, M_p, lq_list, n_lq, lq_cap, lq_kind, lq_next, lq_nothead, hbits, rstart, rend);
}
void launch_lq_bits_count(hipStream_t s, const uint32_t *hbits, uint32_t n_words, uint32_t *wcnt) {
    NP2_LAUNCH(k_lq_bits_count, grid1((uint64_t)n_words + 1), 256, s, hbits, n_words, wcnt);
}
void launch_scatter_regions(hipStream_t s, const uint32_t *hbits, uint32_t n_words, const uint32_t *woff,
                            const uint32_t *rstart, const uint32_t *rend, uint32_t *raw_start, uint32_t *raw_end,
                            uint32_t *n_raw) {
    NP2_LAUNCH(k_scatter_regions, grid1(std::max<uint32_t>(n_words, 1)), 256, s, hbits, n_words, woff, rstart, rend, raw_start, raw_end, n_raw);
}
void launch_lq_merge_flag(hipStream_t s, const uint32_t *raw_start, const uint32_t *raw_end, const uint32_t *n_raw,
                          uint32_t *headflag) {
    NP2_LAUNCH(k_lq_merge_flag, dim3(256), 256, s, raw_start, raw_end, n_raw, headflag);
}
void launch_lq_merge_scan(hipStream_t s, const uint32_t *raw_start, const uint32_t *raw_end, const uint32_t *n_raw, uint32_t n_host,
                          uint32_t *headflag, uint32_t *hidx) {
    NP2_LAUNCH(k_lq_merge_scan, dim3(1), 1024, s, raw_start, raw_end, n_raw, n_host, headflag, hidx);
}
void launch_lq_merge_write(hipStream_t s, const uint32_t *raw_start, const uint32_t *raw_end, const uint32_t *n_raw,
                           const uint32_t *headflag, const uint32_t *hidx, uint32_t *lq_start, uint32_t *lq_end,
                           uint32_t *n_reg) {
    NP2_LAUNCH(k_lq_merge_write, dim3(256), 256, s, raw_start, raw_end, n_raw, headflag, hidx, lq_start, lq_end, n_reg);
}
void launch_read_m(hipStream_t s, const np2_read_t *reads, uint32_t R, const uint8_t *alive, const uint32_t *lq_start,
                   uint32_t n_reg, int32_t *mval) {
    NP2_LAUNCH(k_read_m, grid1(R), 256, s, reads, R, alive, lq_start, n_reg, mval);
}
void launch_pair_count(hipStream_t s, const np2_read_t *reads, uint32_t R, const uint8_t *alive,
                       const uint32_t *lq_start, const uint32_t *lq_end, uint32_t n_reg, const int32_t *smin,
                       uint32_t *pj, uint32_t *pcount, const uint64_t *ck_off, ReadInfo *rinfo) {
    NP2_LAUNCH(k_pair_count, grid1(R), 256, s, reads, R, alive, lq_start, lq_end, n_reg, smin, pj, pcount, ck_off, rinfo);
}
void launch_yak_insert(hipStream_t s, const uint64_t *words, const uint64_t *bucket_off, uint32_t n_buckets,
                       uint64_t max_bucket, uint64_t *table, uint32_t cap_log2, uint32_t *dup_flag, uint32_t gap) {
    uint32_t gx = (uint32_t)((max_bucket + 255) / 256);
    if (gx == 0) gx = 1;
    if (gx > 64) gx = 64;
    hipLaunchKernelGGL(k_yak_insert, dim3(gx, n_buckets), dim3(256), 0, s, words, bucket_off, n_buckets, table,
                       cap_log2, dup_flag, gap);
}
void launch_yak_insert_dup(hipStream_t s, const uint64_t *words, const uint64_t *bucket_off, uint32_t n_buckets,
                           uint64_t max_bucket, uint64_t *table, uint32_t cap_log2, uint32_t *ord, uint32_t gap) {
    uint32_t gx = (uint32_t)((max_bucket + 255) / 256);
    gx = std::min<uint32_t>(64, std::max<uint32_t>(1, gx));
    hipLaunchKernelGGL(k_yak_insert_dup, dim3(gx, n_buckets), dim3(256), 0, s, words, bucket_off, n_buckets, table,
                       cap_log2, ord, gap);
}
void launch_lookup(hipStream_t s, const YakDev &y, const uint64_t *hashes, uint64_t n, uint16_t min_count,
                   uint16_t *out) {
    if (n) NP2_LAUNCH(k_lookup, grid1(n), 256, s, y, hashes, n, min_count, out);
}
void launch_score_strings(hipStream_t s, const YakDev &y, const uint8_t *strs, const uint64_t *off, uint64_t n,
                          uint16_t min_count, uint16_t *out, bool own_strings) {
    if (n) NP2_LAUNCH(k_score_strings, grid1(n * 64), 256, s, y, strs, off, n, min_count, out, own_strings ? 1u : 0u);
}
void launch_cand_score(hipStream_t s, const YakDev &y, const uint32_t *cand_seq_off, const uint8_t *cand_seq,
                       const uint64_t *cand_kmer, const uint32_t *n_cand_p, uint32_t cand_cap, uint16_t min_count,
                       uint16_t *kscore, uint32_t *long_list, uint32_t *n_long) {
    if (!cand_cap) return;
    NP2_LAUNCH(k_cand_score, grid1(cand_cap), 256, s, y, cand_seq_off, cand_kmer, n_cand_p, min_count, kscore, long_list, n_long);
    NP2_LAUNCH(k_cand_score_long, dim3(std::max<uint32_t>(16, std::min<uint32_t>(1024, cand_cap / 4096))), 256, s, y, cand_seq_off, cand_seq, long_list, n_long, min_count, kscore);
}
}
```

### nextpolish2_amd/csrc/np2_kernels.hpp

```cpp
#pragma once
#include <cstddef>
#include <cstdint>
#include <hip/hip_runtime.h>
#include "../../include/np2.h"
#include "np2_lookback.hpp"
#include "np2_launch.hpp"

namespace np2 {

static constexpr uint32_t TILE_SHIFT = 10;
static constexpr uint32_t TILE = 1u << TILE_SHIFT;
static constexpr uint32_t TILE_CAP = 4096;

static constexpr uint32_t DENSE_COLS = 4096;
struct ChunkDesc {
    uint64_t nib_off;
    uint64_t ckbase;
    uint32_t read, ts;
    uint32_t c0, ncols;
    uint32_t first_chunk;
    uint32_t aln_t_e, nck;
    uint32_t pad0;
    uint32_t pad[4];
};
// ... 12 lines not shown
    const int32_t *cov;
    uint32_t L;
    const uint2 *nrec;
    const uint32_t *deep;
    const uint8_t *pflag;
};
struct __attribute__((aligned(16))) ReadInfo {
    uint32_t aln_t_s, n_cols;
    uint32_t nib16;
    uint32_t ck_off;
    uint32_t aln_t_e;
    uint32_t pj, pcount;
    uint32_t pad;
};
struct CandPtrs {
    const np2_read_t *reads;
    const uint8_t *nib;
    const uint64_t *ck_off;
    const uint32_t *ckpt;
    const uint32_t *lq_start;
    const uint32_t *lq_end;
    const uint32_t *pj;
    const uint32_t *pcount;
    const uint8_t *alive;
    const ReadInfo *rinfo;
    const uint32_t *tile_rd_off;
    const uint32_t *tile_rd;
    uint32_t n_tiles;
    uint32_t ksize;
    const uint64_t *rec_key;
    const uint32_t *rec_read;
    const uint32_t *tile_n;
    const uint16_t *rec_pidx;
    uint32_t bucket_cap;
    const uint32_t *refnib;
    uint32_t L;
};
struct YakDev {
    const uint64_t *table;
    uint32_t cap_log2;
    uint32_t k;
    const uint32_t *ord;
};
static constexpr uint64_t YAK_EMPTY = ~0ULL;
#if defined(__HIPCC__)
__device__ __forceinline__ uint16_t yak_get(const YakDev &y, uint64_t x, uint16_t min_count) {
    const uint64_t capm = (1ULL << y.cap_log2) - 1;
    const uint64_t *tb = y.table + ((x & 1023) << y.cap_log2);
    const uint64_t key = x >> 10;
    uint64_t s = key & capm;
    if (y.ord) {
        const uint32_t *ob = y.ord + ((x & 1023) << y.cap_log2);
        uint16_t c = 0;
        int64_t at = -1;
        for (;;) {
            const uint64_t w = tb[s];
            if (w == YAK_EMPTY) return c;
            if ((w >> 10) == key && (uint16_t)(w & 1023) >= min_count && (int64_t)ob[s] > at) at = ob[s], c = (uint16_t)(w & 1023);
            s = (s + 1) & capm;
        }
    }
    for (;;) {
        const uint64_t w = tb[s];
        if (w == YAK_EMPTY) return 0;
        if ((w >> 10) == key) {
            const uint16_t c = (uint16_t)(w & 1023);
            return c >= min_count ? c : 0;
        }
        s = (s + 1) & capm;
    }
}
#endif

void launch_encode_ref(hipStream_t s, const uint8_t *read0, uint32_t L, uint8_t *refnib, uint32_t nbytes, uint32_t stride, uint32_t *err);
void launch_chunk_counts(hipStream_t s, const ChunkDesc *descs, uint32_t n_chunks, const uint8_t *nib, uint64_t *chunk_st, uint32_t epoch);
void launch_diff_reads(hipStream_t s, const ChunkDesc *descs, uint32_t n_chunks, const uint8_t *nib, const uint64_t *refw,
                       const uint8_t *refnib, const uint8_t *refeo, uint32_t eo_stride, uint32_t L, uint64_t *keys, uint32_t *vals, uint32_t *tile_cur,
                       uint32_t n_tiles, uint32_t bucket_cap, uint64_t ovf_base, uint32_t ovf_cap, uint32_t *ovf_cnt,
                       uint32_t *ckpt, uint64_t *chunk_st, uint32_t epoch, uint32_t *err);
void launch_post(hipStream_t s, uint32_t *scal, uint32_t n_scal, uint32_t *mbox, uint32_t seq, uint32_t *d0 = nullptr,
                 const uint32_t *s0 = nullptr, uint32_t *d1 = nullptr, const uint32_t *s1 = nullptr, uint32_t *d2 = nullptr,
                 const uint32_t *s2 = nullptr, uint32_t *d3 = nullptr, const uint32_t *s3 = nullptr,
                 const uint32_t *ends_of = nullptr, uint32_t *ends_dst = nullptr);
void launch_fill(hipStream_t s, uint8_t *p, uint64_t bytes, uint8_t byte);
void launch_copy(hipStream_t s, uint8_t *dst, const uint8_t *src, uint64_t bytes);
void launch_copy_len(hipStream_t s, uint8_t *dst, const uint8_t *src, const uint32_t *n_dev, uint32_t elem, uint64_t cap_bytes);
void launch_copy_counted(hipStream_t s, uint32_t *dst, const uint32_t *src, const uint32_t *n_dev, uint32_t cap, uint32_t words_per = 1);
void launch_init_alive(hipStream_t s, const np2_read_t *reads, uint32_t R, uint8_t *alive);
void launch_kill_reads(hipStream_t s, const uint32_t *ids, uint32_t n, uint8_t *alive);
void launch_revive_reads(hipStream_t s, const uint32_t *ids, uint32_t n, uint8_t *alive);
void launch_kill_flagged(hipStream_t s, const uint8_t *flag, uint32_t n, uint8_t *alive);
void launch_dp_short(hipStream_t s, const GraphPtrs &gp, const void *refw, const uint32_t *run_start,
                     const uint32_t *n_runs, uint32_t max_runs, uint32_t *run_end, int64_t *run_gain, uint32_t *emit,
                     uint32_t *path_begin, uint64_t *path, uint32_t *dp_list, uint32_t *n_dp_list);
void launch_dp_long(hipStream_t s, const GraphPtrs &gp, const uint32_t *run_start, uint32_t max_runs, const uint2 *nrec,
                    int64_t *nscore, uint32_t *nbesti, uint32_t *n0_besti, uint32_t *run_end, int64_t *last_n0_score,
                    int64_t *run_gain, uint32_t *emit, uint32_t *path_begin, uint64_t *path, uint8_t *run_flag,
                    const uint32_t *dp_list, const uint32_t *n_dp_list);
void launch_dp_finish(hipStream_t s, const GraphPtrs &gp, const uint32_t *run_start, const uint32_t *n_runs,
                      const int64_t *nscore, const uint32_t *nbesti, const uint32_t *n0_besti, const int64_t *last_n0_score,
                      unsigned long long *total_gain, uint32_t *blocks_done, uint32_t *best_idx, const int64_t *run_gain,
                      const long long *tile_gain, uint32_t n_tiles, uint32_t *emit, uint32_t *path_begin, uint64_t *path);
void launch_bt_write(hipStream_t s, const GraphPtrs &gp, const uint32_t *run_start, const uint32_t *n_runs,
                     uint32_t run_bound, const uint32_t *emit, const uint32_t *eoff, const uint64_t *path,
                     uint32_t *cns_pos, uint8_t *cns_base, uint8_t *cns_cls, uint8_t *lq_nothead, uint32_t *lqc);
void launch_lq_list(hipStream_t s, const GraphPtrs &gp, const uint32_t *run_start, const uint32_t *n_runs,
                    uint32_t run_bound, const uint32_t *emit, const uint32_t *eoff, const uint64_t *path,
                    const uint32_t *lqoff, uint32_t cap, uint32_t *lq_list, uint32_t *err);
void launch_default_tail(hipStream_t s, const GraphPtrs &gp, const uint32_t *best_idx, const uint32_t *M_p, uint8_t *cns_base,
                         uint8_t *cns_cls, uint32_t *lq_list, uint32_t *n_lq, uint32_t cap, uint32_t *err);
void launch_lq_scan(hipStream_t s, const uint32_t *cns_pos, const uint8_t *cns_base, const uint8_t *cns_cls,
                    const uint32_t *M_p, const uint32_t *lq_list, const uint32_t *n_lq, uint32_t lq_cap, uint8_t *lq_kind,
                    uint32_t *lq_next, uint8_t *lq_nothead, uint32_t *hbits, uint32_t n_hwords, uint32_t *rstart, uint32_t *rend);
void launch_lq_merge_scan_lb(hipStream_t s, const Lookback &lb, const uint32_t *raw_start, const uint32_t *raw_end, const uint32_t *n_raw,
                             uint32_t n_host, uint32_t *headflag, uint32_t *hidx, uint32_t *err);
uint32_t lq_merge_lb_blocks();
void launch_lq_merge_scan(hipStream_t s, const uint32_t *raw_start, const uint32_t *raw_end, const uint32_t *n_raw, uint32_t n_host,
                          uint32_t *headflag, uint32_t *hidx);
void launch_scan_lb_popc(hipStream_t s, const Lookback &lb, const uint32_t *bits, uint32_t *out, uint32_t n_words, uint32_t *err);
void launch_lq_bits_count(hipStream_t s, const uint32_t *hbits, uint32_t n_words, uint32_t *wcnt);
void launch_scatter_regions(hipStream_t s, const uint32_t *hbits, uint32_t n_words, const uint32_t *woff,
                            const uint32_t *rstart, const uint32_t *rend, uint32_t *raw_start, uint32_t *raw_end,
                            uint32_t *n_raw);
void launch_lq_merge_flag(hipStream_t s, const uint32_t *raw_start, const uint32_t *raw_end, const uint32_t *n_raw,
                          uint32_t *headflag);
void launch_lq_merge_write(hipStream_t s, const uint32_t *raw_start, const uint32_t *raw_end, const uint32_t *n_raw,
                           const uint32_t *headflag, const uint32_t *hidx, uint32_t *lq_start, uint32_t *lq_end,
                           uint32_t *n_reg);
void launch_read_m(hipStream_t s, const np2_read_t *reads, uint32_t R, const uint8_t *alive, const uint32_t *lq_start,
                   uint32_t n_reg, int32_t *mval);
void launch_yak_insert(hipStream_t s, const uint64_t *words, const uint64_t *bucket_off, uint32_t n_buckets,
                       uint64_t max_bucket, uint64_t *table, uint32_t cap_log2, uint32_t *dup_flag, uint32_t gap = 0);
void launch_yak_insert_dup(hipStream_t s, const uint64_t *words, const uint64_t *bucket_off, uint32_t n_buckets,
                           uint64_t max_bucket, uint64_t *table, uint32_t cap_log2, uint32_t *ord, uint32_t gap = 0);
void launch_lookup(hipStream_t s, const YakDev &y, const uint64_t *hashes, uint64_t n, uint16_t min_count, uint16_t *out);
void launch_score_strings(hipStream_t s, const YakDev &y, const uint8_t *strs, const uint64_t *off, uint64_t n,
                          uint16_t min_count, uint16_t *out, bool own_strings);
void launch_cand_score(hipStream_t s, const YakDev &y, const uint32_t *cand_seq_off, const uint8_t *cand_seq,
                       const uint64_t *cand_kmer, const uint32_t *n_cand_p, uint32_t cand_cap, uint16_t min_count,
                       uint16_t *kscore, uint32_t *long_list, uint32_t *n_long);


void launch_pair_count(hipStream_t s, const np2_read_t *reads, uint32_t R, const uint8_t *alive,
                       const uint32_t *lq_start, const uint32_t *lq_end, uint32_t n_reg, const int32_t *smin,
                       uint32_t *pj, uint32_t *pcount, const uint64_t *ck_off, ReadInfo *rinfo);
void launch_scan_lb_excl(hipStream_t s, const Lookback &lb, const uint32_t *in, uint32_t *out, uint32_t n, bool write_end,
                          uint32_t *err);
uint32_t scan_lb_blocks(uint64_t n);
void launch_scan_small_excl(hipStream_t s, const uint32_t *in, uint32_t *out, uint32_t n, const uint32_t *n_dev,
                            uint32_t *total_out, bool write_end);
void launch_scan_small_incl(hipStream_t s, const int32_t *in, int32_t *out, uint32_t n, const uint32_t *n_dev);
void launch_scan_small_min(hipStream_t s, const int32_t *in, int32_t *out, uint32_t n, const uint32_t *n_dev);
void launch_region_measure(hipStream_t s, const CandPtrs &c, uint32_t n_reg, uint32_t *kept_read, uint32_t *kept_len,
                           uint32_t *kept_col, uint32_t *reg_ncand, uint32_t *reg_bytes, uint32_t *reg_maxlen,
                           uint32_t *blk_sum);
uint32_t cand_offsets_blocks(uint32_t n_reg);
void launch_cand_offsets(hipStream_t s, const uint32_t *blk_sum, uint32_t n_reg, uint32_t *blk_coff, uint32_t *blk_soff,
                         uint32_t *cand_off, uint32_t *reg_soff, uint32_t *n_cand, uint32_t *n_bytes, uint32_t *grow,
                         const Lookback *lb = nullptr, uint32_t *err = nullptr);
void launch_region_write(hipStream_t s, const CandPtrs &c, uint32_t n_reg, const uint32_t *kept_read,
                         const uint32_t *kept_len, const uint32_t *kept_col, const uint32_t *reg_ncand,
                         const uint32_t *reg_bytes, const uint32_t *blk_coff, const uint32_t *blk_soff, uint32_t *cand_off,
                         uint32_t *reg_soff, uint32_t cand_cap, uint32_t seq_cap, uint32_t *cand_order, uint64_t *cand_kmer,
                         uint32_t *cand_seq_off, uint8_t *cand_seq);

uint32_t tile_scan_blocks(uint32_t n_tiles);
void launch_tile_layout(hipStream_t s, uint32_t *tile_cur, uint32_t n_tiles, uint32_t bucket_cap, uint32_t *tile_n,
                        uint32_t *tile_scan, uint32_t *tile_scanb, const uint32_t *ovf_cnt, uint32_t *out,
                        const Lookback *lb = nullptr, uint32_t *err = nullptr);
void launch_tile_sort(hipStream_t s, uint16_t *pidx, const np2_read_t *reads, const uint8_t *nib, const uint32_t *tile_n,
                      uint32_t n_tiles, uint32_t bucket_cap, uint32_t max_tile, uint64_t *keys, uint32_t *vals,
                      uint32_t *err);
void launch_gather_buckets(hipStream_t s, const np2_read_t *reads, const uint8_t *nib, const uint32_t *tile_n,
                           const uint32_t *tile_scanb, uint32_t n_tiles, uint32_t bucket_cap, const uint64_t *bkeys,
                           const uint32_t *bvals, uint64_t *keys, uint32_t *vals);
void launch_gather_spill(hipStream_t s, const np2_read_t *reads, const uint8_t *nib, const uint64_t *okeys,
                         const uint32_t *ovals, uint32_t n, uint64_t *keys, uint32_t *vals);
void launch_tile_count(hipStream_t s, const uint64_t *keys, const uint32_t *vals, const uint32_t *tile_n,
                       const uint32_t *tile_scan, uint32_t bucket_cap, uint32_t n_tiles, const uint8_t *alive,
                       uint32_t *tile_nn, uint32_t *tile_nr);
void launch_tile_offsets(hipStream_t s, const uint32_t *tile_nn, const uint32_t *tile_nr, uint32_t n_tiles,
                         uint32_t *tile_noff, uint32_t *tile_roff, uint32_t *n_nodes, uint32_t *n_runs, uint32_t *reset,
                         uint32_t n_reset, const Lookback *lb = nullptr, uint32_t *err = nullptr,
                         const long long *tile_gain = nullptr, unsigned long long *gain_total = nullptr);
void launch_tile_write(hipStream_t s, const uint64_t *keys, const uint32_t *vals, const uint32_t *tile_n,
                       const uint32_t *tile_scan, uint32_t bucket_cap, const uint32_t *tile_noff, const uint32_t *tile_roff,
                       uint32_t n_tiles, const uint8_t *alive, uint32_t L, NodeArrays nd, uint2 *nrec, uint32_t *node_off,
                       uint32_t *run_start, const np2_read_t *reads, const uint32_t *tile_rd_off, const uint32_t *tile_rd,
                       int32_t *cov, const uint8_t *refnib, uint32_t *emit, long long *tile_gain, uint32_t *deep_flag, uint32_t deep_min,
                       uint8_t *pflag);

static constexpr uint32_t PF_CAP = 960;
static constexpr uint32_t PF_HALO = 64;
static constexpr uint32_t PF_CAP_MID = 2048;
static constexpr uint32_t PF_CAP_BIG = 3584;
static constexpr uint32_t PF_COV_MAX = 8192;
static constexpr uint32_t PF_REDO = 1u;
static constexpr uint32_t PF_NEED_BIG = 2u;
struct PfTile {
    const uint64_t *keys;
    const uint32_t *vals;
    const uint32_t *tile_n, *tile_scan;
    const uint16_t *pidx;
    const uint8_t *alive;
    const np2_read_t *reads;
    const uint32_t *tile_rd_off, *tile_rd;
    const uint8_t *refnib;
    uint16_t *slots;
    uint32_t *tile_cnt, *tile_lq;
    long long *tile_gain;
    uint32_t *flags, *n_bad, *bad_list, *n_bad2, *bad_list2;
    long long *end_rel;
    unsigned long long *gain_total;
    unsigned long long *prof;
    uint32_t L, n_tiles, bucket_cap;
    uint32_t cap_lim, cap_lim_big, halo_lim, cov_max;
    uint32_t big_enabled;
};
uint64_t pf_slot_entries(uint32_t n_tiles, uint64_t T);
void launch_pf_tile(hipStream_t s, const PfTile &a);
void launch_pf_compact(hipStream_t s, uint32_t n_tiles, const uint16_t *slots, const uint32_t *tile_scan, const uint32_t *tile_cnt,
                       const uint32_t *tile_coff, const uint32_t *tile_lqoff, uint32_t *cns_pos, uint8_t *cns_base,
                       uint8_t *cns_cls, uint8_t *lq_nothead, uint32_t *lq_list, uint32_t lq_cap, uint32_t *err, uint32_t *flags,
                       uint32_t *flags_out, uint32_t *n_bad, uint32_t *n_bad2);

struct RegionTables {
    const uint32_t *cand_off;
    const uint32_t *order;
    uint16_t *kscore;
    const uint32_t *seq_off;
    const uint8_t *seq;
    uint32_t n_reg;
};
struct RechPtrs {
    const void *groups;
    const uint32_t *job_off;
    const uint32_t *rech;
    const uint32_t *cand_off;
    const uint32_t *keep_list;
    const uint32_t *seq_off;
    const uint8_t *seq;
    const uint8_t *cns_base;
    uint32_t n_groups;
};
void launch_vote_phase(hipStream_t s, const RegionTables &rt, bool asref, bool use_all, const uint32_t *lq_start,
                       uint32_t own_lo, uint32_t own_hi, uint8_t *reg_lable, uint8_t *grp, uint32_t *ecount, int32_t *ref_w,
                       uint8_t *ref_seen, uint8_t *bad, uint32_t *first_reg, uint32_t *err);
// ... 76 lines not shown
```

### nextpolish2_amd/csrc/np2_regions.hip

```cpp
#include "np2_common.hpp"
#include "np2_kernels.hpp"
#include "np2_blockscan.hpp"
#include "np2_lookback.hpp"

namespace np2 {

static constexpr uint8_t LB_TEMP = 0x01, LB_SUCC = 0x80, LB_HETE = 0x40, LB_RECH = 0x20;

__device__ __forceinline__ uint32_t min_support(uint32_t n) { return n >= 9 ? 3u : (n >= 6 ? 2u : 1u); }

struct SubWave {
    uint32_t base;
    bool half;
    __device__ __forceinline__ uint64_t ballot(bool p) const {
        const uint64_t b = __ballot(p);
        return half ? (b >> base) & 0xFFFFFFFFull : b;
    }
    template <class T> __device__ __forceinline__ T shfl(T v, uint32_t j) const { return __shfl(v, (int)(base + j)); }
};

struct WaveStats {
    uint64_t eqmask;
    uint32_t stat;
    uint32_t c;
// ... 873 lines not shown
                                                      uint32_t *__restrict__ n_groups, uint32_t *__restrict__ n_jobs,
                                                      uint32_t *__restrict__ err) {
    __shared__ uint32_t sh[8];
    const uint32_t bid = lb_block_id(lb, sh);
    const uint32_t n_rech = *n_rech_p;
    uint32_t hj[LB_REG_ITEMS], hs = 0, js = 0;
#pragma unroll
    for (uint32_t k = 0; k < LB_REG_ITEMS; ++k) {
        const uint32_t e = (bid * 256 + threadIdx.x) * LB_REG_ITEMS + k;
        hj[k] = e < n_rech ? head_jobs[e] : 0u;
        hs += hj[k] ? 1u : 0u;
        js += hj[k] ? hj[k] - 1u : 0u;
    }
    uint32_t nh, nj, pre_h, pre_j;
    uint32_t lh = block_excl_scan<OpAdd, 4>(hs, sh, nh);
    uint32_t lj = block_excl_scan<OpAdd, 4>(js, sh, nj);
    lb_exclusive2(lb, bid, nh, nj, sh, err, pre_h, pre_j);
    if (pre_j + nj < pre_j) atomicOr(err, 128u);
#pragma unroll
    for (uint32_t k = 0; k < LB_REG_ITEMS; ++k) {
        if (!hj[k]) continue;
        const uint32_t e = (bid * 256 + threadIdx.x) * LB_REG_ITEMS + k;
        groups[pre_h + lh] = tmp_groups[e];
        job_off[pre_h + lh] = pre_j + lj;
        ++lh;
        lj += hj[k] - 1u;
    }
    if (bid == n_blocks - 1 && threadIdx.x == 0) {
        *n_groups = pre_h + nh;
        *n_jobs = pre_j + nj;
        job_off[pre_h + nh] = pre_j + nj;
    }
}

struct RechCtx {
    const RechGroup *groups;
    const uint32_t *job_off;
    const uint32_t *rech;
    const uint32_t *cand_off;
    const uint32_t *keep_list;
    const uint32_t *seq_off;
    const uint8_t *seq;
    const uint8_t *cns_base;
    uint32_t n_groups;
};
__device__ __forceinline__ uint32_t job_group(const RechCtx &cx, uint32_t job) {
    uint32_t lo = 0, hi = cx.n_groups;
    while (lo < hi) {
        const uint32_t mid = (lo + hi) >> 1;
        if (cx.job_off[mid] <= job) lo = mid + 1; else hi = mid;
    }
    return lo - 1;
}
template <bool WRITE> __device__ uint32_t rech_string(const RechCtx &cx, uint32_t job, uint8_t *__restrict__ out) {
    const uint32_t gi = job_group(cx, job);
    const RechGroup &G = cx.groups[gi];
    uint32_t rem = job - cx.job_off[gi];
    uint32_t pick[6];
    for (uint32_t x = G.n; x-- > 0;) {
        pick[x] = rem % G.lens[x];
        rem /= G.lens[x];
    }
    uint32_t o = 0;
    for (uint32_t i = G.sl; i < G.el; ++i, ++o)
        if (WRITE) out[o] = cx.cns_base[i];
    for (uint32_t x = 0; x < G.n; ++x) {
        const uint32_t g = cx.rech[G.first + x];
        const uint32_t c = cx.keep_list[cx.cand_off[g] + pick[x]];
        const uint32_t so = cx.seq_off[c], len = cx.seq_off[c + 1] - so;
        for (uint32_t t = 0; t < len; ++t, ++o)
            if (WRITE) out[o] = cx.seq[so + t];
        if (x + 1 < G.n)
            for (uint32_t i = G.bs[x]; i < G.be[x]; ++i, ++o)
                if (WRITE) out[o] = cx.cns_base[i];
    }
    for (uint32_t i = G.sr; i < G.er; ++i, ++o)
        if (WRITE) out[o] = cx.cns_base[i];
    return o;
}
__device__ __forceinline__ void k_rech_job_len(const uint32_t np2_bid, const uint32_t np2_nb, RechCtx cx, uint32_t n_jobs, uint32_t *__restrict__ len) {
    uint32_t j = np2_bid * blockDim.x + threadIdx.x;
    if (j < n_jobs) len[j] = rech_string<false>(cx, j, nullptr);
}
__device__ __forceinline__ void k_rech_job_build(const uint32_t np2_bid, const uint32_t np2_nb, RechCtx cx, uint32_t n_jobs, const uint64_t *__restrict__ soff,
                                 uint8_t *__restrict__ blob) {
    uint32_t j = np2_bid * blockDim.x + threadIdx.x;
    if (j < n_jobs) rech_string<true>(cx, j, blob + soff[j]);
}
__device__ __forceinline__ void k_u32_to_u64_off(const uint32_t np2_bid, const uint32_t np2_nb, const uint32_t *__restrict__ in, uint32_t n, uint64_t *__restrict__ out) {
    uint32_t i = np2_bid * blockDim.x + threadIdx.x;
    if (i < n) out[i] = in[i];
}

__device__ __forceinline__ void k_rech_apply(const uint32_t np2_bid, const uint32_t np2_nb, RechCtx cx, const uint16_t *__restrict__ score, uint16_t *__restrict__ keep_ks) {
    uint32_t gi = np2_bid * blockDim.x + threadIdx.x;
    if (gi >= cx.n_groups) return;
    const RechGroup &G = cx.groups[gi];
    const uint32_t j0 = cx.job_off[gi];
    if (G.n == 1) {
        const uint32_t g = cx.rech[G.first];
        for (uint32_t t = 0; t < G.lens[0]; ++t) keep_ks[cx.cand_off[g] + t] = score[j0 + t];
        return;
    }
    for (uint32_t x = 0; x < G.n; ++x) {
        const uint32_t g = cx.rech[G.first + x];
        for (uint32_t t = 0; t < G.lens[x]; ++t) keep_ks[cx.cand_off[g] + t] = 0;
    }
    for (uint32_t j = 0; j < G.njobs; ++j) {
        const uint16_t ks = score[j0 + j];
        if (!ks) continue;
        uint32_t rem = j;
        for (uint32_t x = G.n; x-- > 0;) {
            const uint32_t p = rem % G.lens[x];
            rem /= G.lens[x];
            keep_ks[cx.cand_off[cx.rech[G.first + x]] + p] = ks;
        }
    }
}

__device__ __forceinline__ void k_rech_select(const uint32_t np2_bid, const uint32_t np2_nb, const uint32_t *__restrict__ rech, const uint32_t *__restrict__ n_rech_p,
                              const uint32_t *__restrict__ cand_off, const uint32_t *__restrict__ keep_n,
                              const uint32_t *__restrict__ keep_list, const uint16_t *__restrict__ keep_ks,
                              const uint32_t *__restrict__ order, uint32_t first_yak, uint8_t *__restrict__ reg_lable,
                              uint32_t *__restrict__ seed_cand) {
    uint32_t e = np2_bid * blockDim.x + threadIdx.x;
    if (e >= *n_rech_p) return;
    const uint32_t g = rech[e], c0 = cand_off[g], n = keep_n[g];
    uint32_t c = 0, valid = 0;
    for (uint32_t p = 0; p < n; ++p)
        if (keep_ks[c0 + p] != 0) {
            if (c == 0 || order[keep_list[c0 + p]] == 0) c = p + 1;
            ++valid;
        }
    if (valid > 1) reg_lable[g] |= LB_TEMP;
    if (c != 0) {
        seed_cand[g] = keep_list[c0 + c - 1];
    } else if (first_yak) {
        uint32_t i = 0;
        for (uint32_t p = 0; p < n; ++p)
            if (order[keep_list[c0 + p]] == 0) {
                i = p;
                break;
            }
        seed_cand[g] = keep_list[c0 + i];
    }
}
__device__ __forceinline__ void k_rech_relabel(const uint32_t np2_bid, const uint32_t np2_nb, uint8_t *__restrict__ reg_lable, uint32_t n_reg) {
    uint32_t g = np2_bid * blockDim.x + threadIdx.x;
    if (g >= n_reg) return;
    const uint8_t l = reg_lable[g];
    if (!(l & LB_RECH)) return;
    reg_lable[g] = (l & LB_TEMP) ? (uint8_t)(l ^ LB_TEMP) : (uint8_t)(l ^ LB_RECH);
}

__device__ __forceinline__ void k_vote_counts(const uint32_t np2_bid, const uint32_t np2_nb, const uint32_t *__restrict__ first_reg, const uint8_t *__restrict__ bad,
                                                      uint32_t R, uint32_t *__restrict__ out) {
    __shared__ uint32_t sk[16], sb[16];
    uint32_t nk = 0, nb = 0;
    for (uint32_t r = threadIdx.x; r < R; r += 1024) {
        nk += first_reg[r] != 0xFFFFFFFFu ? 1u : 0u;
        nb += bad[r] ? 1u : 0u;
    }
    for (int o = 32; o > 0; o >>= 1) {
        nk += __shfl_xor(nk, o);
        nb += __shfl_xor(nb, o);
    }
    if ((threadIdx.x & 63) == 0) {
        sk[threadIdx.x >> 6] = nk;
        sb[threadIdx.x >> 6] = nb;
    }
    __syncthreads();
    if (threadIdx.x == 0) {
        uint32_t a = 0, b = 0;
        for (int i = 0; i < 16; ++i) {
            a += sk[i];
            b += sb[i];
        }
        out[0] = a;
        out[1] = b;
    }
}

static inline dim3 g1(uint64_t n, uint32_t bs = 256) { return dim3((unsigned)((n + bs - 1) / bs)); }

void launch_vote_phase(hipStream_t s, const RegionTables &rt, bool asref, bool use_all, const uint32_t *lq_start,
                       uint32_t own_lo, uint32_t own_hi, uint8_t *reg_lable, uint8_t *grp, uint32_t *ecount, int32_t *ref_w,
                       uint8_t *ref_seen, uint8_t *bad, uint32_t *first_reg, uint32_t *err) {
    if (rt.n_reg)
        NP2_LAUNCH(k_vote_phase, g1((uint64_t)((rt.n_reg + 1) / 2) * 64), 256, s, rt, asref ? 1u : 0u, use_all ? 1u : 0u, lq_start, own_lo, own_hi, reg_lable, grp, ecount, ref_w, ref_seen, bad, first_reg, err);
}
void launch_vote_counts(hipStream_t s, const uint32_t *first_reg, const uint8_t *bad, uint32_t R, uint32_t *out) {
    NP2_LAUNCH(k_vote_counts, dim3(1), 1024, s, first_reg, bad, R, out);
}
void launch_edges_write(hipStream_t s, const RegionTables &rt, const uint8_t *reg_lable, const uint8_t *grp,
                        const uint32_t *ecount, const uint32_t *eoff, uint64_t *ekey, uint32_t *eval) {
    if (rt.n_reg)
        NP2_LAUNCH(k_edges_write, g1((uint64_t)rt.n_reg * 64), 256, s, rt, reg_lable, grp, ecount, eoff, ekey, eval);
}
void launch_edges_row(hipStream_t s, const RegionTables &rt, const uint8_t *grp, const uint32_t *ecount, const uint32_t *pj,
                      const uint32_t *pcount, const uint8_t *alive, uint32_t R, uint32_t *band, uint32_t *row_n, uint32_t *ovf) {
    if (R) NP2_LAUNCH(k_edges_row, g1((uint64_t)R * 64), 256, s, rt, grp, ecount, pj, pcount, alive, R, band, row_n, ovf);
}
void launch_vote_rows_count(hipStream_t s, const uint32_t *band, const uint32_t *row_n, const uint8_t *bad, bool use_all, uint32_t R,
                            uint32_t *cnt, uint32_t *nokey) {
    if (R) NP2_LAUNCH(k_vote_rows_count, g1((uint64_t)R * 64), 256, s, band, row_n, bad, use_all ? 1u : 0u, R, cnt, nokey);
}
void launch_vote_rows_emit(hipStream_t s, const uint32_t *band, const uint32_t *row_n, const uint8_t *bad, bool use_all,
                           const uint32_t *first_reg, uint32_t R, const uint32_t *off, void *edges, uint32_t *n_out, uint32_t *nokey) {
    if (R) NP2_LAUNCH(k_vote_rows_emit, g1((uint64_t)R * 64), 256, s, band, row_n, bad, use_all ? 1u : 0u, first_reg, R, off, (uint2 *)edges, n_out, nokey);
}
void launch_band_emit(hipStream_t s, const uint32_t *band, uint32_t R, const uint32_t *row_off, uint64_t *ukey, uint32_t *uw,
                      uint32_t *n_out, uint64_t key_add) {
    if (R) NP2_LAUNCH(k_band_emit, g1((uint64_t)R * 64), 256, s, band, R, row_off, ukey, uw, n_out, key_add);
}
void launch_edge_reduce(hipStream_t s, const uint64_t *ekey, const uint32_t *eval, uint32_t n, uint32_t *flag,
                        uint32_t *wout) {
    if (n) NP2_LAUNCH(k_edge_reduce, g1(n), 256, s, ekey, eval, n, flag, wout);
}
void launch_edge_compact(hipStream_t s, const uint64_t *ekey, const uint32_t *flag, const uint32_t *idx,
                         const uint32_t *wout, uint32_t n, uint64_t *ukey, uint32_t *uw, uint32_t *n_out) {
    if (n) NP2_LAUNCH(k_edge_compact, g1(n), 256, s, ekey, flag, idx, wout, n, ukey, uw, n_out);
}
void launch_seed(hipStream_t s, const RegionTables &rt, int32_t max_indel_len, uint8_t *reg_lable, uint32_t *seed_cand,
                 uint32_t *keep_n, uint32_t *keep_list, uint16_t *keep_ks, uint32_t *err) {
    if (rt.n_reg)
        NP2_LAUNCH(k_seed, g1((uint64_t)((rt.n_reg + 1) / 2) * 64), 256, s, rt, max_indel_len, reg_lable, seed_cand, keep_n, keep_list, keep_ks, err);
}
uint32_t region_lb_blocks(uint32_t n_reg) { return (n_reg + 256 * LB_REG_ITEMS - 1) / (256 * LB_REG_ITEMS); }
void launch_splice_find(hipStream_t s, const uint32_t *cns_pos, const uint32_t *M_p, const uint32_t *lq_start,
                        const uint32_t *lq_end, const uint8_t *reg_lable, uint8_t lable, uint32_t n_reg,
                        uint32_t *idx_s, uint32_t *idx_e, uint32_t *stuck) {
    NP2_LAUNCH(k_splice_find, g1(n_reg), 256, s, cns_pos, M_p, lq_start, lq_end, reg_lable, lable, n_reg, idx_s, idx_e, stuck);
}
void launch_splice_plan(hipStream_t s, const Lookback &lb, const uint8_t *reg_lable, uint8_t lable, uint32_t n_reg,
                        const uint32_t *stuck, const uint32_t *idx_s, const uint32_t *idx_e, const uint32_t *seed_cand,
                        const uint32_t *seq_off, uint32_t *ap_g, uint32_t *ap_s, uint32_t *ap_e, int32_t *ap_delta,
                        int32_t *ap_shift_incl, uint32_t *n_ap, const uint32_t *M_in, uint32_t *M_out, uint32_t out_cap, uint32_t *err) {
    const uint32_t nb = region_lb_blocks(n_reg);
    NP2_LAUNCH(k_splice_plan, dim3(nb), 256, s, lb, nb, reg_lable, lable, n_reg, stuck, idx_s, idx_e, seed_cand, seq_off, ap_g, ap_s, ap_e, ap_delta, ap_shift_incl, n_ap, M_in, M_out, out_cap, err);
}
void launch_splice_write(hipStream_t s, const uint32_t *in_pos, const uint8_t *in_base, const uint32_t *M_p, uint32_t M_cap,
                         const uint32_t *ap_g, const uint32_t *ap_s, const uint32_t *ap_e, const int32_t *ap_delta,
                         const int32_t *ap_shift_incl, const uint32_t *n_ap, uint32_t max_ap, const uint32_t *lq_start,
                         const uint32_t *seed_cand, const uint32_t *seq_off, const uint8_t *seq, uint32_t *out_pos,
                         uint8_t *out_base) {
    NP2_LAUNCH(k_splice_bases, dim3((M_cap + SPLICE_SPAN - 1) / SPLICE_SPAN), 256, s, in_pos, in_base, M_p, ap_s, ap_e, ap_shift_incl, n_ap, out_pos, out_base);
    if (max_ap)
        NP2_LAUNCH(k_splice_seeds, g1((uint64_t)max_ap * 8, 256), 256, s, ap_g, ap_s, ap_delta, ap_shift_incl, n_ap, lq_start, seed_cand, seq_off, seq, out_pos, out_base);
}
void launch_shard_bounds(hipStream_t s, const uint32_t *cns_pos, const uint32_t *M_p, const uint32_t *t, uint32_t *out) {
    NP2_LAUNCH(k_shard_bounds, dim3(1), 64, s, cns_pos, M_p, t[0], t[1], t[2], t[3], t[4], t[5], out);
}
void launch_rech_list(hipStream_t s, const Lookback &lb, const uint8_t *reg_lable, uint32_t n_reg, uint32_t *rech,
                      uint32_t *n_rech, unsigned long long *blob_bound, uint32_t *err) {
    const uint32_t nb = region_lb_blocks(n_reg);
    NP2_LAUNCH(k_rech_list, dim3(nb), 256, s, lb, nb, reg_lable, n_reg, rech, n_rech, blob_bound, err);
}
void launch_rech_groups(hipStream_t s, const Lookback &lb, const uint32_t *rech, const uint32_t *n_rech_p, uint32_t max_rech,
                        const uint32_t *cns_pos, const uint32_t *M_p, const uint32_t *lq_start, const uint32_t *lq_end,
                        const uint32_t *keep_n, uint32_t ksize, const uint32_t *reg_maxlen, void *tmp_groups,
                        uint32_t *head_jobs, void *groups, uint32_t *job_off, uint32_t *n_groups, uint32_t *n_jobs,
                        unsigned long long *blob_bound, uint32_t *err) {
    NP2_LAUNCH(k_rech_groups, dim3((max_rech + 255) / 256), 256, s, rech, n_rech_p, cns_pos, M_p, lq_start, lq_end, keep_n, ksize, reg_maxlen, (RechGroup *)tmp_groups, head_jobs, blob_bound, err);
    const uint32_t nb = region_lb_blocks(max_rech);
    NP2_LAUNCH(k_rech_compact, dim3(nb), 256, s, lb, nb, n_rech_p, head_jobs, (const RechGroup *)tmp_groups, (RechGroup *)groups, job_off, n_groups, n_jobs, err);
}
size_t rech_group_bytes() { return sizeof(RechGroup); }
static RechCtx mk_rech(const RechPtrs &p) {
    return RechCtx{(const RechGroup *)p.groups, p.job_off, p.rech, p.cand_off, p.keep_list, p.seq_off, p.seq,
                   p.cns_base, p.n_groups};
}
void launch_rech_job_len(hipStream_t s, const RechPtrs &p, uint32_t n_jobs, uint32_t *len) {
    if (n_jobs) NP2_LAUNCH(k_rech_job_len, g1(n_jobs, 64), 64, s, mk_rech(p), n_jobs, len);
}
void launch_rech_job_build(hipStream_t s, const RechPtrs &p, uint32_t n_jobs, const uint32_t *soff32, uint64_t *soff64,
                           uint8_t *blob) {
    if (!n_jobs) return;
    NP2_LAUNCH(k_u32_to_u64_off, g1(n_jobs + 1), 256, s, soff32, n_jobs + 1, soff64);
    NP2_LAUNCH(k_rech_job_build, g1(n_jobs, 64), 64, s, mk_rech(p), n_jobs, soff64, blob);
}
void launch_rech_apply(hipStream_t s, const RechPtrs &p, const uint16_t *score, uint16_t *keep_ks) {
    if (p.n_groups) NP2_LAUNCH(k_rech_apply, g1(p.n_groups, 64), 64, s, mk_rech(p), score, keep_ks);
}
void launch_rech_select(hipStream_t s, const uint32_t *rech, const uint32_t *n_rech_p, uint32_t max_rech,
                        const uint32_t *cand_off, const uint32_t *keep_n, const uint32_t *keep_list,
                        const uint16_t *keep_ks, const uint32_t *order, bool first_yak, uint8_t *reg_lable,
                        uint32_t *seed_cand) {
    if (max_rech)
        NP2_LAUNCH(k_rech_select, g1(max_rech, 64), 64, s, rech, n_rech_p, cand_off, keep_n, keep_list, keep_ks, order, first_yak ? 1u : 0u, reg_lable, seed_cand);
}
void launch_rech_relabel(hipStream_t s, uint8_t *reg_lable, uint32_t n_reg) {
    NP2_LAUNCH(k_rech_relabel, g1(n_reg), 256, s, reg_lable, n_reg);
}

}
```

Before: 4284.

## Fuse kernel launches across pipeline and fold completion signal into batched post

Scores short candidate k-mers inside the region-write kernel and keeps a separate pass only for long candidates. Also merges the u32-to-u64 offset conversion into the job-build kernel, combines two fills into one split fill, and drops a memset by having vote_counts zero the third scalar. In batched flushes, the final k_post launch now carries the completion-word write, so the separate k_flush_done kernel is skipped when possible, and the done signal is only issued when a waiter needs it. The goal is fewer launches and fewer passes over candidate memory, at the cost of more complex completion bookkeeping, with a device counter that has to be reset after a failure.

```diff
diff --git a/nextpolish2_amd/csrc/np2_batch.cpp b/nextpolish2_amd/csrc/np2_batch.cpp
--- a/nextpolish2_amd/csrc/np2_batch.cpp
+++ b/nextpolish2_amd/csrc/np2_batch.cpp
@@ -52,6 +52,8 @@
     std::string fail_msg;
 
     uint32_t *done_host = nullptr, *done_dev = nullptr;
+    uint32_t *done_ctr = nullptr;
+    bool need_post = false;
     uint32_t done_seq = 0;
     std::atomic<uint32_t> issued_seq{0};
     std::atomic<uint32_t> done_pub{0};
@@ -99,6 +101,11 @@
 
 void flush(np2_batch *b) {
     const int n = (int)b->recs.size();
+    const bool need_post = b->need_post;
+    b->need_post = false;
+    const KernelDesc *const post_kd = post_kernel_desc();
+    bool posted = false;
+    uint32_t seq = 0;
     const double t_begin = now_ms();
     double t_issued = t_begin;
     std::vector<size_t> idx(n, 0);
@@ -145,6 +152,21 @@
                 }
                 if (!best || defer < best_defer || (defer == best_defer && c > best_n)) best = kd, best_n = c, best_defer = defer;
             }
+            uint32_t n_post = 0;
+            if (need_post && best == post_kd) {
+                n_post = 1;
+                for (int i = 0; i < n && n_post; ++i) {
+                    auto &q = b->recs[i].q;
+                    if (idx[i] >= q.size()) continue;
+                    if (q[idx[i]].kd != best || idx[i] + 1 != q.size()) n_post = 0;
+                }
+                if (n_post) {
+                    n_post = 0;
+                    for (int i = 0; i < n; ++i) n_post += idx[i] < b->recs[i].q.size() ? 1u : 0u;
+                    seq = ++b->done_seq;
+                    posted = true;
+                }
+            }
             uint32_t grids[MAXB];
             const void *args[MAXB];
             int m = 0;
@@ -172,6 +194,7 @@
                 auto &r = b->recs[i];
                 if (idx[i] >= r.q.size() || r.q[idx[i]].kd != best) continue;
                 grids[m] = r.q[idx[i]].grid;
+                if (n_post) post_pack_set_completion(r.arena.data() + r.q[idx[i]].arg_off, b->done_dev, seq, b->done_ctr, n_post);
                 args[m] = r.arena.data() + r.q[idx[i]].arg_off;
                 ++m;
                 ++idx[i];
@@ -181,14 +204,17 @@
             issue();
         }
         HIPCHK(hipGetLastError());
-        const uint32_t seq = ++b->done_seq;
-        NP2_LAUNCH(k_flush_done, 1, 64, s, b->done_dev, seq);
+        if (need_post && !posted) {
+            seq = ++b->done_seq;
+            NP2_LAUNCH(k_flush_done, 1, 64, s, b->done_dev, seq);
+        }
         t_issued = now_ms();
-        b->issued_seq.store(seq, std::memory_order_release);
+        if (need_post) b->issued_seq.store(seq, std::memory_order_release);
     } catch (const std::exception &ex) {
         b->fail_msg = ex.what();
         b->failed.store(true);
         (void)hipStreamSynchronize(s);
+        (void)hipMemset(b->done_ctr, 0, sizeof(uint32_t));
         for (np2_ctx *cx : b->slots) cx->lb_dirty = true, cx->h2d_inflight = false;
     }
     tl_recorder() = saved;
@@ -254,6 +280,7 @@
     {
         std::lock_guard<std::mutex> l(b->sync_mu);
         my_gen = b->flush_gen.load(std::memory_order_relaxed);
+        b->need_post |= need_done;
         if (++b->n_waiting == b->n_active) {
             flush(b);
             b->n_waiting = 0;
@@ -334,6 +361,8 @@
         HIPCHK(hipHostMalloc((void **)&b->done_host, 256 * (size_t)(n_slots + 1), hipHostMallocMapped | hipHostMallocCoherent));
         memset(b->done_host, 0, 256 * (size_t)(n_slots + 1));
         HIPCHK(hipHostGetDevicePointer((void **)&b->done_dev, b->done_host, 0));
+        HIPCHK(hipMalloc((void **)&b->done_ctr, 256));
+        HIPCHK(hipMemset(b->done_ctr, 0, 256));
         b->recs.resize(n_slots);
         b->jobs.resize(n_slots);
         for (int i = 0; i < n_slots; ++i) {
@@ -368,6 +397,7 @@
         (void)hipEventDestroy(e.second);
     }
     if (b->done_host) (void)hipHostFree(b->done_host);
+    if (b->done_ctr) (void)hipFree(b->done_ctr);
     if (b->stream) (void)hipStreamDestroy(b->stream);
     delete b;
 }
@@ -432,6 +462,7 @@
                     std::lock_guard<std::mutex> l2(b->sync_mu);
                     b->n_active = m;
                     b->n_waiting = 0;
+                    b->need_post = false;
                     b->failed.store(false);
                 }
                 ++b->job_gen;
diff --git a/nextpolish2_amd/csrc/np2_cand.hip b/nextpolish2_amd/csrc/np2_cand.hip
--- a/nextpolish2_amd/csrc/np2_cand.hip
+++ b/nextpolish2_amd/csrc/np2_cand.hip
@@ -209,7 +209,8 @@
     }
 };
 
-__device__ void cand_write(const CandCtx &cx, uint32_t r, const np2_read_t &rd, uint32_t pj, uint32_t g, uint32_t col, uint32_t t,
+template <class Ctx>
+__device__ void cand_write(const Ctx &cx, uint32_t r, const np2_read_t &rd, uint32_t pj, uint32_t g, uint32_t col, uint32_t t,
                            uint32_t len, uint8_t *__restrict__ seq_out, uint64_t *kmer_out) {
     const uint8_t *base = cx.nib + rd.nib_off;
     const uint32_t limit = cx.lq_end[pj] + cx.ksize;
@@ -677,7 +678,29 @@
     }
 }
 
-__device__ __forceinline__ void k_region_write(const uint32_t np2_bid0, const uint32_t np2_nb, CandCtx cx, uint32_t n_reg, const uint32_t *__restrict__ kept_read,
+struct WriteCtx {
+    const uint8_t *nib;
+    const uint32_t *lq_start;
+    const uint32_t *lq_end;
+    const ReadInfo *rinfo;
+    const uint32_t *refnib;
+    uint32_t ksize;
+    uint32_t n_reg;
+    uint32_t cand_cap;
+    uint32_t seq_cap;
+    uint32_t min_count;
+};
+__device__ __forceinline__ void list_long(bool is_long, uint32_t ci, uint32_t *__restrict__ long_list, uint32_t *__restrict__ n_long) {
+    const uint64_t m = __ballot(is_long);
+    if (m) {
+        const uint32_t lane = threadIdx.x & 63, lead = (uint32_t)__builtin_ctzll(m);
+        uint32_t base = 0;
+        if (lane == lead) base = atomicAdd(n_long, (uint32_t)__builtin_popcountll(m));
+        base = __shfl(base, lead);
+        if (is_long) long_list[base + lanes_below(m)] = ci;
+    }
+}
+__device__ __forceinline__ void k_region_write(const uint32_t np2_bid0, const uint32_t np2_nb, WriteCtx cx, YakDev y, const uint32_t *__restrict__ kept_read,
                                                       const uint32_t *__restrict__ kept_len,
                                                       const uint32_t *__restrict__ kept_col,
                                                       const uint32_t *__restrict__ reg_ncand,
@@ -685,17 +708,20 @@
                                                       const uint32_t *__restrict__ blk_coff,
                                                       const uint32_t *__restrict__ blk_soff,
                                                       uint32_t *__restrict__ cand_off, uint32_t *__restrict__ reg_soff,
-                                                      uint32_t cand_cap,
-                                                      uint32_t seq_cap, uint32_t *__restrict__ cand_order,
+                                                      uint32_t *__restrict__ cand_order,
                                                       uint64_t *__restrict__ cand_kmer, uint32_t *__restrict__ cand_seq_off,
-                                                      uint8_t *__restrict__ cand_seq) {
+                                                      uint8_t *__restrict__ cand_seq, uint16_t *__restrict__ kscore,
+                                                      uint32_t *__restrict__ long_list, uint32_t *__restrict__ n_long) {
     const uint32_t np2_bid = xcd_order(np2_bid0, np2_nb);
     __shared__ __attribute__((aligned(4))) uint8_t s_str[RM_REG][CLEAN_MAX_LEN];
     __shared__ uint64_t s_km[RM_REG];
+    __shared__ uint32_t s_ks[RM_REG];
     __shared__ uint32_t s_so[RM_REG][64];
     __shared__ uint32_t s_oc[RM_REG];
     __shared__ uint32_t s_q[4][RM_RPW * 64];
     const uint32_t lane = threadIdx.x & 63, wv = (uint32_t)__builtin_amdgcn_readfirstlane((int)(threadIdx.x >> 6));
+    const uint32_t n_reg = cx.n_reg, cand_cap = cx.cand_cap, seq_cap = cx.seq_cap;
+    const uint16_t min_count = (uint16_t)cx.min_count;
     const uint32_t g0 = (np2_bid * 4 + wv) * RM_RPW, mb0 = g0 / 4;
     uint32_t nq = 0;
     uint32_t oc = 0, ob = 0;
@@ -739,6 +765,8 @@
         if (ok) {
             cand_order[ci] = rd_[h];
             cand_seq_off[ci] = so;
+        } else if (act && ci < cand_cap) {
+            kscore[ci] = 0;
         }
         const bool clean = ok && col[h] == CAND_CLEAN;
         const uint64_t cm = __ballot(clean);
@@ -756,35 +784,50 @@
         ob += rb[h];
     }
     wave_lds_sync();
-    for (uint32_t e = lane; e < nq; e += 64) {
-        const uint32_t w = s_q[wv][e], slot = w >> 6, li = w & 63;
-        const uint32_t g = (np2_bid * 4 + slot / RM_RPW) * RM_RPW + slot % RM_RPW;
-        const size_t ks = (size_t)g * LQSEQ_MAX_CAN_COUNT + li;
-        const uint32_t r = kept_read[ks], len = kept_len[ks];
-        uint32_t col = kept_col[ks];
-        const ReadInfo ri = cx.rinfo[r];
-        const np2_read_t rd = rinfo_read(ri);
-        const uint32_t t0 = max(cx.lq_start[g], rd.aln_t_s);
-        if (col == CAND_CLEAN) col = t0;
-        const uint32_t ci = s_oc[slot] + li;
-        uint64_t km;
-        cand_write(cx, r, rd, ri.pj, g, col, t0, len, cand_seq + s_so[slot][li], &km);
-        cand_kmer[ci] = km;
-        if (li == 0 && r == 0) s_km[slot] = km;
+    for (uint32_t e0 = 0; e0 < nq; e0 += 64) {
+        const uint32_t e = e0 + lane;
+        bool is_long = false;
+        uint32_t ci = 0;
+        if (e < nq) {
+            const uint32_t w = s_q[wv][e], slot = w >> 6, li = w & 63;
+            const uint32_t g = (np2_bid * 4 + slot / RM_RPW) * RM_RPW + slot % RM_RPW;
+            const size_t ks = (size_t)g * LQSEQ_MAX_CAN_COUNT + li;
+            const uint32_t r = kept_read[ks], len = kept_len[ks];
+            uint32_t col = kept_col[ks];
+            const ReadInfo ri = cx.rinfo[r];
+            const np2_read_t rd = rinfo_read(ri);
+            const uint32_t t0 = max(cx.lq_start[g], rd.aln_t_s);
+            if (col == CAND_CLEAN) col = t0;
+            ci = s_oc[slot] + li;
+            uint64_t km;
+            cand_write(cx, r, rd, ri.pj, g, col, t0, len, cand_seq + s_so[slot][li], &km);
+            if (cand_kmer) cand_kmer[ci] = km;
+            is_long = len > y.k;
+            uint16_t sc = 0;
+            if (!is_long) {
+                if (km != INVALID_KMER) sc = yak_get(y, km, min_count);
+                kscore[ci] = sc;
+            }
+            if (li == 0 && r == 0) s_km[slot] = km, s_ks[slot] = sc;
+        }
+        list_long(is_long, ci, long_list, n_long);
     }
     wave_lds_sync();
 #pragma unroll
     for (uint32_t h = 0; h < RM_RPW; ++h) {
         if (!((clean_h >> h) & 1u)) continue;
         const uint32_t slot = wv * RM_RPW + h;
+        const bool is_long = my_clean[h] && my_len[h] > y.k;
         if (my_clean[h]) {
-            cand_kmer[my_ci[h]] = s_km[slot];
+            if (cand_kmer) cand_kmer[my_ci[h]] = s_km[slot];
+            if (!is_long) kscore[my_ci[h]] = (uint16_t)s_ks[slot];
             typedef uint32_t u32_any __attribute__((aligned(1)));
             uint8_t *dst = cand_seq + my_so[h];
             const uint32_t L4 = my_len[h] & ~3u;
             for (uint32_t j = 0; j < L4; j += 4) *reinterpret_cast<u32_any *>(dst + j) = *reinterpret_cast<const uint32_t *>(&s_str[slot][j]);
             for (uint32_t j = L4; j < my_len[h]; ++j) dst[j] = s_str[slot][j];
         }
+        list_long(is_long, my_ci[h], long_list, n_long);
     }
 }
 
@@ -838,9 +881,13 @@
                          const uint32_t *kept_len, const uint32_t *kept_col, const uint32_t *reg_ncand,
                          const uint32_t *reg_bytes, const uint32_t *blk_coff, const uint32_t *blk_soff, uint32_t *cand_off,
                          uint32_t *reg_soff, uint32_t cand_cap, uint32_t seq_cap, uint32_t *cand_order, uint64_t *cand_kmer,
-                         uint32_t *cand_seq_off, uint8_t *cand_seq) {
+                         uint32_t *cand_seq_off, uint8_t *cand_seq, const YakDev &y, uint16_t min_count, uint16_t *kscore,
+                         uint32_t *long_list, uint32_t *n_long) {
+    static_assert(Sig<decltype(&k_region_write)>::N >= 17, "k_region_write's argument pack has grown: fewer than 17 contigs per batched launch");
+    const WriteCtx w{c.nib, c.lq_start, c.lq_end, c.rinfo, c.refnib, c.ksize, n_reg, cand_cap, seq_cap, min_count};
     if (n_reg)
-        NP2_LAUNCH(k_region_write, dim3((n_reg + RM_REG - 1) / RM_REG), 256, s, mk_cand(c), n_reg, kept_read, kept_len, kept_col, reg_ncand, reg_bytes, blk_coff, blk_soff, cand_off, reg_soff, cand_cap, seq_cap, cand_order, cand_kmer, cand_seq_off, cand_seq);
-}
-
-}
+        NP2_LAUNCH_WAVES(k_region_write, RM_WAVES, dim3((n_reg + RM_REG - 1) / RM_REG), 256, s, w, y,
+                         kept_read, kept_len, kept_col, reg_ncand, reg_bytes, blk_coff, blk_soff, cand_off, reg_soff, cand_order, cand_kmer, cand_seq_off, cand_seq, kscore, long_list, n_long);
+}
+
+}
diff --git a/nextpolish2_amd/csrc/np2_host.cpp b/nextpolish2_amd/csrc/np2_host.cpp
--- a/nextpolish2_amd/csrc/np2_host.cpp
+++ b/nextpolish2_amd/csrc/np2_host.cpp
@@ -236,16 +236,16 @@
         uint32_t *v_first = (uint32_t *)vbuf;
         int32_t *v_refw = (int32_t *)(vbuf + RP * 4);
         uint8_t *v_seen = vbuf + RP * 8, *v_bad = vbuf + RP * 9;
-        op_fill(cx, v_first, 0xFF, RP * 4);
-        op_fill(cx, v_refw, 0, RP * 6);
+        launch_fill_split(s, vbuf, RP * 10, RP * 4, 0xFF, 0);
         launch_vote_phase(s, rt, asref, use_all, cx->lq_start.p, own_lo, own_hi, cx->reg_lable.p, cx->grp.p, cx->ecount.p,
                           v_refw, v_seen, v_bad, v_first, cx->scal.p + S_ERR);
         exclusive_total_n(cx, cx->ecount.p, cx->eoff.p, n_reg);
+        static_assert(S_M2 == S_M1 + 1 && S_M3 == S_M1 + 2, "k_vote_counts writes these three");
         launch_vote_counts(s, v_first, v_bad, R, cx->scal.p + S_M1);
         cx->band.ensure(band_words + 4);
         cx->band_n.ensure((size_t)R + 2);
-        op_fill(cx, cx->scal.p + S_M3, 0, 4);
-        launch_edges_row(s, rt, cx->grp.p, cx->ecount.p, cx->pj.p, cx->pcount.p, cx->alive.p, R, cx->band.p, cx->band_n.p,
+        launch_edges_row(
+s, rt, cx->grp.p, cx->ecount.p, cx->pj.p, cx->pcount.p, cx->alive.p, R, cx->band.p, cx->band_n.p,
                          cx->scal.p + S_M3);
         if (wide) {
             exclusive_total_n(cx, cx->band_n.p, row_off, R);
@@ -279,12 +279,12 @@
             sc = fetch_scal(cx, cx->scal.p + S_M0, cx->eoff.p + n_reg);
         } else {
             pin = (uint8_t *)cx->pin_d2h.ensure(b_v + b_off + (size_t)likely * EB + 64);
+            op_d2h(cx, pin, cx->votepack.p, b_v + b_off);
+            launch_copy_counted(cx->stream, (uint32_t *)(pin + b_v + b_off), (const uint32_t *)(cx->votepack.p + b_v + b_off),
+                                (const uint32_t *)(cx->votepack.p + b_v) + R, likely * (uint32_t)(EB / 4), (uint32_t)(EB / 4));
             const uint32_t seq = ++cx->mbox_seq;
             launch_post(cx->stream, cx->scal.p, S_COUNT, cx->mbox_dev, seq, cx->scal.p + S_M0, cx->eoff.p + n_reg, nullptr, nullptr,
                         nullptr, nullptr, nullptr, nullptr, nullptr, nullptr);
-            op_d2h(cx, pin, cx->votepack.p, b_v + b_off);
-            launch_copy_counted(cx->stream, (uint32_t *)(pin + b_v + b_off), (const uint32_t *)(cx->votepack.p + b_v + b_off),
-                                (const uint32_t *)(cx->votepack.p + b_v) + R, likely * (uint32_t)(EB / 4), (uint32_t)(EB / 4));
             op_sync(cx);
             if (__atomic_load_n(&cx->mbox_host[0], __ATOMIC_ACQUIRE) != seq)
                 throw Np2Error(NP2_E_DEVICE, "mailbox not posted after a synchronisation");
@@ -1005,7 +1005,7 @@
     cx->kept_len.ensure((size_t)NC_cap + 2);
     cx->kept_col.ensure((size_t)NC_cap + 2);
     cx->cand_order.ensure((size_t)NC_cap + 2);
-    cx->cand_kmer.ensure((size_t)NC_cap + 2);
+    if (cx->trace) cx->cand_kmer.ensure((size_t)NC_cap + 2);
     cx->cand_seq_off.ensure((size_t)NC_cap + 2);
     if (!exact_bytes) cx->cand_seq.ensure((size_t)SB_cap + 64);
     cx->kscore.ensure((size_t)NC_cap + 2);
@@ -1040,12 +1040,14 @@
         }
         launch_region_write(s, cp, n_reg, cx->kept_read.p, cx->kept_len.p, cx->kept_col.p, cx->reg_ncand.p,
                             cx->reg_bytes.p, cx->blk_coff.p, cx->blk_soff.p, cx->cand_off.p, cx->reg_soff.p, NC_cap + 1,
-                            SB_cap, cx->cand_order.p, cx->cand_kmer.p, cx->cand_seq_off.p, cx->cand_seq.p);
+                            SB_cap, cx->cand_order.p, cx->trace ? cx->cand_kmer.p : nullptr, cx->cand_seq_off.p,
+                            cx->cand_seq.p, cx->yaks[0].dev(), min_kmer_count, cx->kscore.p, cx->long_list.p,
+                            cx->scal.p + S_NLONG);
     }
     {
         EventTimer t(cx, "kmer_score");
-        launch_cand_score(s, cx->yaks[0].dev(), cx->cand_seq_off.p, cx->cand_seq.p, cx->cand_kmer.p, cx->scal.p + S_NC,
-                          NC_cap, min_kmer_count, cx->kscore.p, cx->long_list.p, cx->scal.p + S_NLONG);
+        launch_cand_score_long(s, cx->yaks[0].dev(), cx->cand_seq_off.p, cx->cand_seq.p, NC_cap, min_kmer_count,
+                               cx->kscore.p, cx->long_list.p, cx->scal.p + S_NLONG);
     }
     pc.n_reg = n_reg;
     pc.NC_cap = NC_cap;
@@ -1079,9 +1081,6 @@
     std::vector<uint32_t> sc;
     if (cx->sink_dst && cx->sink_cap) launch_copy_len(cx->stream, cx->sink_dst, dbase, M_p, 1, cx->sink_cap);
     if (r.want_bases || r.want_pos) {
-        const uint32_t seq = ++cx->mbox_seq;
-        launch_post(cx->stream, cx->scal.p, S_COUNT, cx->mbox_dev, seq, cx->scal.p + S_M0, M_p, nullptr, nullptr, nullptr, nullptr,
-                    nullptr, nullptr, dpos, cx->scal.p + S_M1);
         if (r.want_bases) r.bases = (uint8_t *)pinned_pool().get((size_t)M_cap + 1);
         if (r.want_pos) r.pos = (uint32_t *)pinned_pool().get(((size_t)M_cap + 1) * 4);
         if ((r.want_bases && !r.bases) || (r.want_pos && !r.pos)) throw Np2Error(NP2_E_NOMEM, "pinned result allocation failed");
@@ -1091,6 +1090,9 @@
         if (r.want_bases && !exact_b) op_d2h(cx, r.bases, dbase, first);
         if (r.want_pos && !exact_p) op_d2h(cx, r.pos, dpos, (size_t)first * 4);
         if ((exact_b || !r.want_bases) && (exact_p || !r.want_pos)) first = M_cap;
+        const uint32_t seq = ++cx->mbox_seq;
+        launch_post(cx->stream, cx->scal.p, S_COUNT, cx->mbox_dev, seq, cx->scal.p + S_M0, M_p, nullptr, nullptr, nullptr, nullptr,
+                    nullptr, nullptr, dpos, cx->scal.p + S_M1);
         op_sync(cx);
         if (__atomic_load_n(&cx->mbox_host[0], __ATOMIC_ACQUIRE) != seq)
             throw Np2Error(NP2_E_DEVICE, "mailbox not posted after a synchronisation");
diff --git a/nextpolish2_amd/csrc/np2_kernels.hip b/nextpolish2_amd/csrc/np2_kernels.hip
--- a/nextpolish2_amd/csrc/np2_kernels.hip
+++ b/nextpolish2_amd/csrc/np2_kernels.hip
@@ -30,7 +30,8 @@
                        uint32_t *__restrict__ dst0, const uint32_t *__restrict__ src0, uint32_t *__restrict__ dst1,
                        const uint32_t *__restrict__ src1, uint32_t *__restrict__ dst2, const uint32_t *__restrict__ src2,
                        uint32_t *__restrict__ dst3, const uint32_t *__restrict__ src3,
-                       const uint32_t *__restrict__ ends_of, uint32_t *__restrict__ ends_dst) {
+                       const uint32_t *__restrict__ ends_of, uint32_t *__restrict__ ends_dst,
+                       uint32_t *__restrict__ done_word, uint32_t done_seq, uint32_t *__restrict__ done_ctr, uint32_t done_n) {
     if (threadIdx.x == 0) {
         if (dst0) *dst0 = *src0;
         if (dst1) *dst1 = *src1;
@@ -47,6 +48,15 @@
         mbox[1 + threadIdx.x] = __hip_atomic_load(&scal[threadIdx.x], __ATOMIC_RELAXED, __HIP_MEMORY_SCOPE_AGENT);
     __threadfence_system();
     if (threadIdx.x == 0) __hip_atomic_store(&mbox[0], seq, __ATOMIC_RELEASE, __HIP_MEMORY_SCOPE_SYSTEM);
+    if (done_word && threadIdx.x == 0) {
+        __threadfence_system();
+        const uint32_t before = __hip_atomic_fetch_add(done_ctr, 1u, __ATOMIC_ACQ_REL, __HIP_MEMORY_SCOPE_AGENT);
+        if (before + 1 == done_n) {
+            __hip_atomic_store(done_ctr, 0u, __ATOMIC_RELAXED, __HIP_MEMORY_SCOPE_AGENT);
+            __threadfence_system();
+            __hip_atomic_store(done_word, done_seq, __ATOMIC_RELEASE, __HIP_MEMORY_SCOPE_SYSTEM);
+        }
+    }
 }
 __device__ __forceinline__ void k_fill(const uint32_t np2_bid, const uint32_t np2_nb, uint8_t *__restrict__ p, uint64_t n, uint32_t v4) {
     const uint64_t o = ((uint64_t)np2_bid * 256 + threadIdx.x) * 16;
@@ -55,6 +65,17 @@
         *reinterpret_cast<uint4 *>(p + o) = make_uint4(v4, v4, v4, v4);
     } else {
         for (uint64_t i = o; i < min(o + 16, n); ++i) p[i] = (uint8_t)v4;
+    }
+}
+__device__ __forceinline__ void k_fill_split(const uint32_t np2_bid, const uint32_t np2_nb, uint8_t *__restrict__ p, uint64_t n, uint64_t split,
+                                             uint32_t va4, uint32_t vb4) {
+    const uint64_t o = ((uint64_t)np2_bid * 256 + threadIdx.x) * 16;
+    if (o >= n) return;
+    if ((((uintptr_t)p) & 15) == 0 && o + 16 <= n && (o + 16 <= split || o >= split)) {
+        const uint32_t v4 = o < split ? va4 : vb4;
+        *reinterpret_cast<uint4 *>(p + o) = make_uint4(v4, v4, v4, v4);
+    } else {
+        for (uint64_t i = o; i < min(o + 16, n); ++i) p[i] = (uint8_t)(i < split ? va4 : vb4);
     }
 }
 __device__ __forceinline__ void k_copy(const uint32_t np2_bid, const uint32_t np2_nb, uint8_t *__restrict__ dst, const uint8_t *__restrict__ src, uint64_t n) {
@@ -1283,30 +1304,6 @@
     if ((threadIdx.x & 63) == 0) out[w] = sc;
 }
 
-__device__ __forceinline__ void k_cand_score(const uint32_t np2_bid, const uint32_t np2_nb, YakDev y, const uint32_t *__restrict__ cand_seq_off, const uint64_t *__restrict__ cand_kmer,
-                             const uint32_t *__restrict__ n_cand_p, uint16_t min_count,
-                             uint16_t *__restrict__ kscore, uint32_t *__restrict__ long_list,
-                             uint32_t *__restrict__ n_long) {
-    const uint32_t c = np2_bid * blockDim.x + threadIdx.x;
-    const bool live = c < *n_cand_p;
-    const uint32_t len = live ? cand_seq_off[c + 1] - cand_seq_off[c] : 0u;
-    const bool is_long = live && len > y.k;
-    const uint64_t m = __ballot(is_long);
-    if (m) {
-        const uint32_t lane = threadIdx.x & 63, lead = (uint32_t)__builtin_ctzll(m);
-        uint32_t base = 0;
-        if (lane == lead) base = atomicAdd(n_long, (uint32_t)__builtin_popcountll(m));
-        base = __shfl(base, lead);
-        if (is_long) long_list[base + (uint32_t)__builtin_popcountll(m & ((1ULL << lane) - 1ULL))] = c;
-    }
-    if (!live) return;
-    uint16_t sc = 0;
-    if (!is_long) {
-        const uint64_t km = cand_kmer[c];
-        if (km != INVALID_KMER) sc = yak_get(y, km, min_count);
-    }
-    kscore[c] = sc;
-}
 __device__ __forceinline__ void k_cand_score_long(const uint32_t np2_bid, const uint32_t np2_nb, YakDev y, const uint32_t *__restrict__ cand_seq_off,
                                   const uint8_t *__restrict__ cand_seq, const uint32_t *__restrict__ long_list,
                                   const uint32_t *__restrict__ n_long, uint16_t min_count,
@@ -1332,10 +1329,23 @@
 void launch_post(hipStream_t s, uint32_t *scal, uint32_t n_scal, uint32_t *mbox, uint32_t seq, uint32_t *d0,
                  const uint32_t *s0, uint32_t *d1, const uint32_t *s1, uint32_t *d2, const uint32_t *s2, uint32_t *d3,
                  const uint32_t *s3, const uint32_t *ends_of, uint32_t *ends_dst) {
-    NP2_LAUNCH(k_post, dim3(1), 64, s, scal, n_scal, mbox, seq, d0, s0, d1, s1, d2, s2, d3, s3, ends_of, ends_dst);
+    NP2_LAUNCH(k_post, dim3(1), 64, s, scal, n_scal, mbox, seq, d0, s0, d1, s1, d2, s2, d3, s3, ends_of, ends_dst,
+               (uint32_t *)nullptr, 0u, (uint32_t *)nullptr, 0u);
+}
+using PostSig = Sig<decltype(&k_post)>;
+const KernelDesc *post_kernel_desc() { return PostSig::desc<64, &k_post, 0>("k_post"); }
+void post_pack_set_completion(void *pack, uint32_t *done_word, uint32_t done_seq, uint32_t *done_ctr, uint32_t done_n) {
+    PostSig::pack_t &p = *static_cast<PostSig::pack_t *>(pack);
+    const_cast<uint32_t *&>(PackGet<14, PostSig::pack_t>::get(p)) = done_word;
+    const_cast<uint32_t &>(PackGet<15, PostSig::pack_t>::get(p)) = done_seq;
+    const_cast<uint32_t *&>(PackGet<16, PostSig::pack_t>::get(p)) = done_ctr;
+    const_cast<uint32_t &>(PackGet<17, PostSig::pack_t>::get(p)) = done_n;
 }
 void launch_fill(hipStream_t s, uint8_t *p, uint64_t bytes, uint8_t byte) {
     if (bytes) NP2_LAUNCH(k_fill, grid1((bytes + 15) / 16), 256, s, p, bytes, 0x01010101u * byte);
+}
+void launch_fill_split(hipStream_t s, uint8_t *p, uint64_t bytes, uint64_t split, uint8_t byte_a, uint8_t byte_b) {
+    if (bytes) NP2_LAUNCH(k_fill_split, grid1((bytes + 15) / 16), 256, s, p, bytes, split, 0x01010101u * byte_a, 0x01010101u * byte_b);
 }
 void launch_copy(hipStream_t s, uint8_t *dst, const uint8_t *src, uint64_t bytes) {
     if (bytes) NP2_LAUNCH(k_copy, grid1((bytes + 15) / 16), 256, s, dst, src, bytes);
@@ -1456,11 +1466,10 @@
                           uint16_t min_count, uint16_t *out, bool own_strings) {
     if (n) NP2_LAUNCH(k_score_strings, grid1(n * 64), 256, s, y, strs, off, n, min_count, out, own_strings ? 1u : 0u);
 }
-void launch_cand_score(hipStream_t s, const YakDev &y, const uint32_t *cand_seq_off, const uint8_t *cand_seq,
-                       const uint64_t *cand_kmer, const uint32_t *n_cand_p, uint32_t cand_cap, uint16_t min_count,
-                       uint16_t *kscore, uint32_t *long_list, uint32_t *n_long) {
+void launch_cand_score_long(hipStream_t s, const YakDev &y, const uint32_t *cand_seq_off, const uint8_t *cand_seq,
+                            uint32_t cand_cap, uint16_t min_count, uint16_t *kscore, const uint32_t *long_list,
+                            const uint32_t *n_long) {
     if (!cand_cap) return;
-    NP2_LAUNCH(k_cand_score, grid1(cand_cap), 256, s, y, cand_seq_off, cand_kmer, n_cand_p, min_count, kscore, long_list, n_long);
     NP2_LAUNCH(k_cand_score_long, dim3(std::max<uint32_t>(16, std::min<uint32_t>(1024, cand_cap / 4096))), 256, s, y, cand_seq_off, cand_seq, long_list, n_long, min_count, kscore);
 }
 }
diff --git a/nextpolish2_amd/csrc/np2_kernels.hpp b/nextpolish2_amd/csrc/np2_kernels.hpp
--- a/nextpolish2_amd/csrc/np2_kernels.hpp
+++ b/nextpolish2_amd/csrc/np2_kernels.hpp
@@ -118,7 +118,10 @@
                  const uint32_t *s0 = nullptr, uint32_t *d1 = nullptr, const uint32_t *s1 = nullptr, uint32_t *d2 = nullptr,
                  const uint32_t *s2 = nullptr, uint32_t *d3 = nullptr, const uint32_t *s3 = nullptr,
                  const uint32_t *ends_of = nullptr, uint32_t *ends_dst = nullptr);
+const KernelDesc *post_kernel_desc();
+void post_pack_set_completion(void *pack, uint32_t *done_word, uint32_t done_seq, uint32_t *done_ctr, uint32_t done_n);
 void launch_fill(hipStream_t s, uint8_t *p, uint64_t bytes, uint8_t byte);
+void launch_fill_split(hipStream_t s, uint8_t *p, uint64_t bytes, uint64_t split, uint8_t byte_a, uint8_t byte_b);
 void launch_copy(hipStream_t s, uint8_t *dst, const uint8_t *src, uint64_t bytes);
 void launch_copy_len(hipStream_t s, uint8_t *dst, const uint8_t *src, const uint32_t *n_dev, uint32_t elem, uint64_t cap_bytes);
 void launch_copy_counted(hipStream_t s, uint32_t *dst, const uint32_t *src, const uint32_t *n_dev, uint32_t cap, uint32_t words_per = 1);
@@ -172,9 +175,9 @@
 void launch_lookup(hipStream_t s, const YakDev &y, const uint64_t *hashes, uint64_t n, uint16_t min_count, uint16_t *out);
 void launch_score_strings(hipStream_t s, const YakDev &y, const uint8_t *strs, const uint64_t *off, uint64_t n,
                           uint16_t min_count, uint16_t *out, bool own_strings);
-void launch_cand_score(hipStream_t s, const YakDev &y, const uint32_t *cand_seq_off, const uint8_t *cand_seq,
-                       const uint64_t *cand_kmer, const uint32_t *n_cand_p, uint32_t cand_cap, uint16_t min_count,
-                       uint16_t *kscore, uint32_t *long_list, uint32_t *n_long);
+void launch_cand_score_long(hipStream_t s, const YakDev &y, const uint32_t *cand_seq_off, const uint8_t *cand_seq,
+                            uint32_t cand_cap, uint16_t min_count, uint16_t *kscore, const uint32_t *long_list,
+                            const uint32_t *n_long);
 
 
 void launch_pair_count(hipStream_t s, const np2_read_t *reads, uint32_t R, const uint8_t *alive,
@@ -198,7 +201,8 @@
                          const uint32_t *kept_len, const uint32_t *kept_col, const uint32_t *reg_ncand,
                          const uint32_t *reg_bytes, const uint32_t *blk_coff, const uint32_t *blk_soff, uint32_t *cand_off,
                          uint32_t *reg_soff, uint32_t cand_cap, uint32_t seq_cap, uint32_t *cand_order, uint64_t *cand_kmer,
-                         uint32_t *cand_seq_off, uint8_t *cand_seq);
+                         uint32_t *cand_seq_off, uint8_t *cand_seq, const YakDev &y, uint16_t min_count, uint16_t *kscore,
+                         uint32_t *long_list, uint32_t *n_long);
 
 uint32_t tile_scan_blocks(uint32_t n_tiles);
 void launch_tile_layout(hipStream_t s, uint32_t *tile_cur, uint32_t n_tiles, uint32_t bucket_cap, uint32_t *tile_n,
diff --git a/nextpolish2_amd/csrc/np2_regions.hip b/nextpolish2_amd/csrc/np2_regions.hip
--- a/nextpolish2_amd/csrc/np2_regions.hip
+++ b/nextpolish2_amd/csrc/np2_regions.hip
@@ -979,14 +979,14 @@
     uint32_t j = np2_bid * blockDim.x + threadIdx.x;
     if (j < n_jobs) len[j] = rech_string<false>(cx, j, nullptr);
 }
-__device__ __forceinline__ void k_rech_job_build(const uint32_t np2_bid, const uint32_t np2_nb, RechCtx cx, uint32_t n_jobs, const uint64_t *__restrict__ soff,
-                                 uint8_t *__restrict__ blob) {
+__device__ __forceinline__ void k_rech_job_build(const uint32_t np2_bid, const uint32_t np2_nb, RechCtx cx, uint32_t n_jobs, const uint32_t *__restrict__ soff32,
+                                 uint64_t *__restrict__ soff64, uint8_t *__restrict__ blob) {
     uint32_t j = np2_bid * blockDim.x + threadIdx.x;
-    if (j < n_jobs) rech_string<true>(cx, j, blob + soff[j]);
-}
-__device__ __forceinline__ void k_u32_to_u64_off(const uint32_t np2_bid, const uint32_t np2_nb, const uint32_t *__restrict__ in, uint32_t n, uint64_t *__restrict__ out) {
-    uint32_t i = np2_bid * blockDim.x + threadIdx.x;
-    if (i < n) out[i] = in[i];
+    if (j >= n_jobs) return;
+    const uint32_t o = soff32[j];
+    soff64[j] = o;
+    if (j == n_jobs - 1) soff64[n_jobs] = soff32[n_jobs];
+    rech_string<true>(cx, j, blob + o);
 }
 
 __device__ __forceinline__ void k_rech_apply(const uint32_t np2_bid, const uint32_t np2_nb, RechCtx cx, const uint16_t *__restrict__ score, uint16_t *__restrict__ keep_ks) {
@@ -1075,6 +1075,7 @@
         }
         out[0] = a;
         out[1] = b;
+        out[2] = 0;
     }
 }
 
@@ -1173,8 +1174,7 @@
 void launch_rech_job_build(hipStream_t s, const RechPtrs &p, uint32_t n_jobs, const uint32_t *soff32, uint64_t *soff64,
                            uint8_t *blob) {
     if (!n_jobs) return;
-    NP2_LAUNCH(k_u32_to_u64_off, g1(n_jobs + 1), 256, s, soff32, n_jobs + 1, soff64);
-    NP2_LAUNCH(k_rech_job_build, g1(n_jobs, 64), 64, s, mk_rech(p), n_jobs, soff64, blob);
+    NP2_LAUNCH(k_rech_job_build, g1(n_jobs, 64), 64, s, mk_rech(p), n_jobs, soff32, soff64, blob);
 }
 void launch_rech_apply(hipStream_t s, const RechPtrs &p, const uint16_t *score, uint16_t *keep_ks) {
     if (p.n_groups) NP2_LAUNCH(k_rech_apply, g1(p.n_groups, 64), 64, s, mk_rech(p), score, keep_ks);
```

After: 4246. No clear change (-0.9%).
